# AlibabaResearch/efficientteacher

Hardware: AMD Instinct MI355X
Metric: SSOD images/sec (teacher+student step) YOLOv5l 640px (higher is better)
Workload: dtype bf16

## Files before the change

### efficientteacher_amd/_lib.py

```python
import ctypes
import os
from ctypes import c_char_p, c_double, c_float, c_int, c_int64, c_size_t, c_void_p

import torch

_HERE = os.path.dirname(os.path.abspath(__file__))
LIB_PATH = os.environ.get("ET_HIP_LIB") or os.path.join(_HERE, "libet_hip.so")

ET_F32, ET_BF16, ET_F16 = 0, 1, 2

P = c_void_p
SIGNATURES = {
    "et_build_arch": (c_char_p, []),
    "et_abi_version": (c_int, []),
    "et_nms_ssod_workspace_bytes": (c_int, [c_int, c_int, ctypes.POINTER(c_size_t)]),
    "et_nms_workspace_bytes": (c_int, [c_int, c_int, c_int, c_int, c_int, ctypes.POINTER(c_size_t)]),
    "et_nms": (c_int, [P, c_int, c_int, c_int, c_float, c_float, c_int, c_int, ctypes.c_uint64, ctypes.c_uint64, c_int,
                       c_float, c_int, P, P, P, P, P, c_size_t, P]),
    "et_nms_ssod": (c_int, [P, c_int, c_int, c_int, c_float, c_float, c_int, c_int, P, P, P, P, P, c_size_t, P]),
    "et_val_match": (c_int, [P, c_int, P, c_int, c_int, P, c_int, P, c_int, c_int, P, c_int, c_int, c_int, c_int64, c_int64,
                             P, P, P, P, P, P]),
    "et_val_ap_workspace_bytes": (c_int, [c_int, ctypes.POINTER(c_size_t)]),
    "et_val_ap": (c_int, [P, P, P, c_int64, P, c_int, c_int, P, P, P, P, P, c_size_t, P]),
    "et_detect_decode": (c_int, [P, c_int, c_int, c_int, c_int, c_int, c_int, c_int64, c_int64, c_int64, c_int64,
                                 P, c_float, P, c_int64, c_int64, P]),
    "et_ema_update": (c_int, [P, P, c_int64, c_float, c_float, P]),
    "et_adamw": (c_int, [P, P, P, P, P, c_int, c_int64, c_float, c_float, c_float, c_float, c_float, c_int, c_float, P, P]),
    "et_adamw_tick": (c_int, [P, c_float, c_float, P, P]),
    "et_adamw_dev": (c_int, [P, P, P, P, P, c_int, c_int64, c_float, c_float, c_float, c_float, c_float, P, c_float, P, P]),
    "et_sgd_nesterov": (c_int, [P, P, P, P, c_int, c_int64, c_float, c_float, c_float, c_int, c_float, P, P]),
    "et_cast_f32_to_lp": (c_int, [P, P, c_int, c_int64, P]),
    "et_scaler_check": (c_int, [P, c_int64, P, P]),
    "et_scaler_update": (c_int, [P, c_float, c_float, c_int, P]),
    "et_ema_update_dev": (c_int, [P, P, c_int64, P, P]),
    "et_sgd_nesterov_dev": (c_int, [P, P, P, P, c_int, c_int64, P, c_int, P, P]),
    "et_conv2d_stats_rows": (c_int, [c_int, c_int, c_int]),
    "et_conv2d_stats_rows_for": (c_int, [c_int] * 12),
    "et_conv2d_stats_adds_for": (c_int, [c_int] * 12),
    "et_conv2d_fwd": (c_int, [P, P, P, c_int] + [c_int] * 11 + [P, P, c_int, P, c_int, P, c_int, P, P]),
    "et_conv2d_dgrad": (c_int, [P, P, P, c_int] + [c_int] * 11 + [c_int, P, c_int, P, P]),
    "et_conv2d_dgrad_bn": (c_int, [P, P, P, c_int] + [c_int] * 10 + [P, c_int, P, c_int, P, P, c_int, P, c_int, P, P]),
    "et_conv2d_wgrad": (c_int, [P, P, P, c_int] + [c_int] * 11 + [P, P]),
    "et_conv2d_wgrad_grouped": (c_int, [P, c_int, c_int] + [c_int] * 9 + [P, P]),
    "et_weight_transpose_all": (c_int, [P, P, c_int, P, c_int, ctypes.c_longlong, P]),
    "et_weight_transpose": (c_int, [P, P, c_int, c_int, c_int, c_int, P]),
    "et_conv2d_kernel_name": (c_int, [c_int] * 13 + [c_char_p, c_int]),
    "et_env_knobs": (c_int, [c_char_p, c_int]),
    "et_colsum": (c_int, [P, c_int, c_int, c_int, c_int, P, P]),
    "et_bn_reduce_rows": (c_int, [c_int, c_int, c_int]),
    "et_bn_finalize": (c_int, [P, c_int, c_int, c_double, P, P, c_float, c_float, P, P, P, P, P, P, P, P]),
    "et_bn_eval_affine": (c_int, [c_int, P, P, P, P, c_float, P, P, P]),
    "et_bn_act_fwd": (c_int, [P, c_int, P, c_int, P, c_int, c_int, c_int, c_int, P, P, c_int, P]),
    "et_bn_act_fwd_sharded": (c_int, [P, c_int, P, c_int, P, c_int, c_int, c_int, c_int, P, c_int, c_double, P, P, c_float, c_float,
                                      P, P, P, P, P, P, c_int, P]),
    "et_bn_act_bwd_sharded": (c_int, [P, c_int, P, c_int, P, c_int, c_int, c_int, c_int, P, P, P, P, P, c_int, P, P, P, c_int, c_int, P]),
    "et_bn_act_bwd": (c_int, [P, c_int, P, c_int, P, c_int, c_int, c_int, c_int, P, P, P, P, P, c_int, P, P, P, P,
                              c_size_t, P]),
    "et_bn_act_bwd_from_partials": (c_int, [P, c_int, P, c_int, P, c_int, c_int, c_int, c_int, P, P, P, P, P, c_int, P, P, P,
                                            P, c_int, P, P]),
    "et_act_bwd": (c_int, [P, c_int, P, c_int, P, c_int, c_int, c_int, c_int, c_int, P]),
    "et_pack_input": (c_int, [P, P, c_int, c_int, c_int, c_int, c_int, P]),
    "et_pack_input_u8": (c_int, [P, P, c_int, c_int, c_int, c_int, c_int, c_float, P]),
    "et_maxpool5_fwd": (c_int, [P, c_int, P, c_int, P, c_int, c_int, c_int, c_int, c_int, P]),
    "et_maxpool5_bwd": (c_int, [P, c_int, P, P, c_int, P, c_int, c_int, c_int, c_int, c_int, c_int, P]),
    "et_upsample2x_fwd": (c_int, [P, c_int, P, c_int, c_int, c_int, c_int, c_int, c_int, P]),
    "et_upsample2x_bwd": (c_int, [P, c_int, P, c_int, c_int, c_int, c_int, c_int, c_int, c_int, P]),
    "et_strong_view_u8": (c_int, [P, P, c_int, c_int, c_int, P, P, P, P, c_int, P]),
    "et_mosaic4_u8": (c_int, [P, P, c_int, c_int, c_int, P]),
    "et_pseudo_label_transform": (c_int, [P, P, P, c_int, c_int, c_int, c_int, c_int, P, P, P]),
    "et_score_log_append": (c_int, [P, P, c_int, c_int, P, P, P, c_int64, P]),
    "et_yolo_loss": (c_int, [P, P]),
    "et_ota_workspace_bytes": (c_int, [c_int, c_int, c_int, c_int, ctypes.POINTER(c_size_t)]),
    "et_ota_assign": (c_int, [P, P, c_float, c_int, P, P, P]),
    "et_select_targets": (c_int, [P, P, c_int, P, P, c_int, c_int, P, P]),
    "et_scale_cast": (c_int, [P, P, c_int, c_int64, c_float, P, P]),
    "et_domain_focal": (c_int, [P, c_int, c_int, c_int64, c_int, c_float, P, c_int, P, P]),
    "et_scale_inplace": (c_int, [P, c_int, c_int64, c_float, P, P]),
    "et_v8_decode": (c_int, [P, c_int, P, c_int, c_int, c_int, c_int, c_int, c_int, c_int, c_float, c_float, P, c_int64, c_int64, P]),
    "et_tal_loss": (c_int, [P, P, P, P, P, P, P, c_int, c_int, c_int, c_int, c_int, c_float, c_float, c_float, P, P, P, P, P]),
    "et_tal_assign_workspace_bytes": (c_int, [c_int, c_int, c_int, ctypes.POINTER(c_size_t)]),
    "et_tal_assign": (c_int, [P, P, P, P, P, P, c_int, c_int, c_int, c_int, c_int, c_float, c_float, c_float, P, P, P, P, P, c_size_t, P]),
    "et_tal_targets_pad": (c_int, [P, c_int, c_int, c_int, c_float, c_float, P, P, P]),
    "et_tal_pseudo_split": (c_int, [P, P, P, P, c_int, c_int, c_int, c_int, c_int, c_int, c_float, c_float, P, P, P, P, P, P, P, P, P]),
    "et_tal_assigned_gt": (c_int, [P, c_int, c_int, c_int, P, P]),
    "et_tal_merge_pseudo": (c_int, [P, P, P, P, P, P, P, P, P, c_int, c_int, c_int, c_int, P, P, P, P]),
}



class WgradItem(ctypes.Structure):
    _fields_ = [("x", ctypes.c_void_p), ("dy", ctypes.c_void_p), ("dw", ctypes.c_void_p), ("ldx", ctypes.c_int),
                ("ldy", ctypes.c_int)]


class LossLevel(ctypes.Structure):
    _fields_ = [("p", P), ("dp", P), ("tobj_ws", P), ("sb", c_int64), ("sa", c_int64), ("sy", c_int64),
                ("sx", c_int64), ("ny", c_int), ("nx", c_int), ("anchors", c_float * 6), ("balance", c_float)]


class LossDesc(ctypes.Structure):
    _fields_ = [("dtype", c_int), ("B", c_int), ("na", c_int), ("nc", c_int), ("NT", c_int), ("nl", c_int),
                ("anchor_t", c_float), ("gr", c_float), ("cp", c_float), ("cn", c_float), ("cls_pw", c_float),
                ("obj_pw", c_float), ("box_w", c_float), ("obj_w", c_float), ("cls_w", c_float),
                ("pass_mask", c_int), ("ignore_obj", c_int), ("targets", P), ("acc_ws", P), ("out", P),
                ("ota_match", P), ("obj_channel", c_int), ("balance_dev", P), ("autobalance_ssi", c_int), ("fl_gamma", c_float), ("level", LossLevel * 4)]


_dll = None
_emulated = False
CALL_TIMER = None
_NO_LAUNCH = frozenset(n for n in (
    "et_build_arch", "et_abi_version", "et_nms_ssod_workspace_bytes", "et_nms_workspace_bytes", "et_conv2d_stats_rows", "et_conv2d_stats_rows_for",
    "et_conv2d_kernel_name", "et_env_knobs", "et_bn_reduce_rows", "et_ota_workspace_bytes", "et_tal_assign_workspace_bytes", "et_val_ap_workspace_bytes"))


class _TimedDll:

    def __init__(self, dll, timer):
        self._dll, self._timer, self._cache = dll, timer, {}

    def __getattr__(self, name):
        fn = self._cache.get(name)
        if fn is None:
            raw = getattr(self._dll, name)
            if name in _NO_LAUNCH or not name.startswith("et_"):
                fn = raw
            else:
                timer = self._timer

                def fn(*a, _raw=raw, _name=name):
                    tok = timer.begin(_name)
                    rc = _raw(*a)
                    timer.end(tok)
                    return rc
            self._cache[name] = fn
        return fn


class EtHipError(RuntimeError):
    pass


def _header_abi_version():
    import re
    with open(os.path.join(os.path.dirname(_HERE), "include", "et_hip.h")) as f:
        m = re.search(r"^#define\s+ET_ABI_VERSION\s+(\d+)", f.read(), re.M)
    if m is None:
        raise EtHipError("include/et_hip.h does not define ET_ABI_VERSION")
    return int(m.group(1))


ABI_VERSION = _header_abi_version()


def _declare(dll):
    for name, (res, args) in SIGNATURES.items():
        fn = getattr(dll, name)
        fn.restype = res
        fn.argtypes = args
    got = dll.et_abi_version()
    if got != ABI_VERSION:
        raise EtHipError(f"{getattr(dll, '_name', 'libet_hip.so')} has ABI version {got}, this binding needs {ABI_VERSION}: "
                         f"rebuild it (python -m efficientteacher_amd.csrc.build)")
    return dll


def load(path=None):
    global _dll
    if _dll is None:
        path = path or LIB_PATH
        if not os.path.exists(path):
            raise EtHipError(
                f"{path} not found: build the gfx950 kernels first "
                f"(python -m efficientteacher_amd.csrc.build).  There is no CPU fallback.")
        _dll = _declare(ctypes.CDLL(path))
    if CALL_TIMER is not None:
        w = getattr(CALL_TIMER, "_wrapped", None)
        if w is None or w._dll is not _dll:
            w = CALL_TIMER._wrapped = _TimedDll(_dll, CALL_TIMER)
        return w
    return _dll


def _use_library_for_tests(path, emulated):
    global _dll, _emulated
    _dll = _declare(ctypes.CDLL(path)) if path else None
    _emulated = bool(emulated) if path else False


def is_emulated():
    return _emulated


def check(rc, what):
    if rc != 0:
        raise EtHipError(f"{what} failed with code {rc}")


def ptr(t):
    if t is None:
        return None
    if not t.is_cuda and not _emulated:
        raise EtHipError("efficientteacher_amd kernels need CUDA/HIP tensors (got a CPU tensor); "
                         "there is no CPU fallback")
    return t.data_ptr()


_RAW_STREAM = getattr(torch._C, "_cuda_getCurrentRawStream", None)


def stream(t=None):
    if _emulated:
        return None
    if _RAW_STREAM is not None:
        idx = t.device.index if t is not None else None
        return _RAW_STREAM(torch.cuda.current_device() if idx is None else idx)
    return torch.cuda.current_stream(t.device if t is not None else None).cuda_stream
```

### efficientteacher_amd/autograd.py

```python
import torch
from torch.autograd import Function

from . import ops

ACT_CODE = {"silu": ops.ACT_SILU, "relu": ops.ACT_RELU, "none": ops.ACT_NONE}

FUSE_BN_BWD = True
FUSE_BN_BWD_K = 1
_RS_DGRAD = {}


def _dgrad_on_rs_tile(cs, x):
    key = (tuple(x.shape), x.dtype, cs.cinp, cs.coutp, cs.k, cs.stride, cs.pad)
    r = _RS_DGRAD.get(key)
    if r is None:
        N, H, W, _ = x.shape
        r = _RS_DGRAD[key] = cs.stride == 1 and ops.kernel_name("dgrad_full", x.dtype, N, H, W, cs.cinp, cs.coutp, cs.k, cs.stride,
                                                               cs.pad).startswith("conv_gemm_rs_kernel")
    return r


def _fuse_into(cs, bn, x=None):
    if bn is None:
        return None
    if FUSE_BN_BWD_K & (1 if cs.k == 1 else 2):
        return bn
    if cs.k > 1 and (FUSE_BN_BWD_K & 4) and x is not None and _dgrad_on_rs_tile(cs, x):
        return bn
    return None
SHARDED_BN = True


def _bn_train_fwd(x, w_lp, cs_stride, cs_pad, bs, act, residual=None, out=None):
    N, IH, IW, Cin = x.shape
    sh = None
    if SHARDED_BN and bs.sh_ld and ops.few_rows("fwd", x.dtype, N, IH, IW, Cin, w_lp.shape[0], w_lp.shape[1], cs_stride, cs_pad):
        sh = bs.acquire_fwd()
    if sh is not None:
        y = ops.conv2d_fwd(x, w_lp, cs_stride, cs_pad, shards=sh)
        N, OH, OW, _ = y.shape
        z, scale, shift, mean, invstd = ops.bn_act_fwd_sharded(y, sh, N * OH * OW, bs.gamma, bs.beta, bs.eps, bs.momentum, bs.rmean,
                                                               bs.rvar, act, residual=residual, out=out)
        return y, z, scale, shift, mean, invstd
    y, stats = ops.conv2d_fwd(x, w_lp, cs_stride, cs_pad, want_stats=True)
    N, OH, OW, _ = y.shape
    scale, shift, mean, invstd = ops.bn_finalize(stats, N * OH * OW, bs.gamma, bs.beta, bs.eps, bs.momentum, bs.rmean, bs.rvar)
    z = ops.bn_act_fwd(y, scale, shift, act, residual=residual, out=out)
    return y, z, scale, shift, mean, invstd


def _bn_sums(y, scale, shift, act, bs):
    return ops.BnBwdSums(y, scale, shift, act, slot=bs if (SHARDED_BN and bs.sh_ld) else None)


def _bn_train_bwd(dz, y, bs, scale, shift, mean, invstd, act, sums=None, out=None):
    part = sums.take(dz) if sums is not None else None
    if SHARDED_BN and bs.sh_ld and (isinstance(part, tuple) or (part is None and ops.few_reduce_rows(y))):
        sh = part if part is not None else bs.acquire_bwd()
        return ops.bn_act_bwd(dz, y, bs.gamma, scale, shift, mean, invstd, act, bs.ggamma, bs.gbeta, out=out, partial=part, shards=sh)
    return ops.bn_act_bwd(dz, y, bs.gamma, scale, shift, mean, invstd, act, bs.ggamma, bs.gbeta, out=out, partial=part)


GRAD_FORK = True

GRAD_READY_HOOK = None


class GradFork:

    def __init__(self):
        self.gb = None
        self.merged = False

    @staticmethod
    def split(x):
        if not (GRAD_FORK and torch.is_grad_enabled() and x.requires_grad):
            return x, x, None
        h = GradFork()
        a, b = _ForkFn.apply(x, h)
        return a, b, h

    @staticmethod
    def tap(b, fork):
        return b if fork is None else _TapFn.apply(b, fork)

    def take(self, shape, dtype):
        g = self.gb
        if g is None or tuple(g.shape) != tuple(shape) or g.dtype != dtype or g.dim() != 4 or g.stride(3) != 1:
            return None
        ld = g.stride(2)
        if not (ld >= g.shape[3] and g.stride(1) == ld * g.shape[2] and g.stride(0) == ld * g.shape[2] * g.shape[1]):
            return None
        return g


class _ForkFn(Function):
    @staticmethod
    def forward(ctx, x, holder):
        ctx.holder = holder
        return (x.as_strided(x.size(), x.stride(), x.storage_offset()), x.as_strided(x.size(), x.stride(), x.storage_offset()))

    @staticmethod
    def backward(ctx, ga, gb):
        h = ctx.holder
        merged = h.merged
        h.gb, h.merged = None, False
        if ga is None or gb is None:
            return (gb if ga is None else ga), None
        if merged:
            return ga, None
        return ga + gb, None


class _TapFn(Function):
    @staticmethod
    def forward(ctx, x, holder):
        ctx.holder = holder
        return x.as_strided(x.size(), x.stride(), x.storage_offset())

    @staticmethod
    def backward(ctx, g):
        ctx.holder.gb = g
        ctx.holder.merged = False
        return g, None


def _wgrad(x, dy, cs, *more_slots):
    hook = GRAD_READY_HOOK
    slots = (cs,) + more_slots

    def done():
        if hook is not None:
            for s in slots:
                hook(s)
    ops.WGRAD_QUEUE.submit(x, dy, cs.gw if not more_slots else _fused_gw(cs), cs.k, cs.stride, cs.pad,
                           on_done=done if hook is not None else None)


def _fused_gw(cs1):
    return cs1.gw.as_strided((2 * cs1.cout, 1, 1, cs1.cinp), (cs1.cinp, cs1.cinp, cs1.cinp, 1), cs1.gw.storage_offset())


class ConvBnActFn(Function):

    @staticmethod
    def forward(ctx, x, residual, wparam, cs, bs, act, nbt, dst=None, bn_in=None, bn_out=None, acc=None):
        ctx.w_needs_grad = wparam.requires_grad
        ctx.bn_in = bn_in if (bn_in is not None and cs.stride == 1 and residual is None) else None
        ctx.acc = acc
        if nbt is not None:
            nbt.add_(1)
        out = None if dst is None else dst[0][..., dst[1]:dst[1] + cs.coutp]
        y, z, scale, shift, mean, invstd = _bn_train_fwd(x, cs.w_lp, cs.stride, cs.pad, bs, act, residual=residual, out=out)
        ctx.cs, ctx.bs, ctx.act = cs, bs, act
        ctx.has_res = residual is not None
        ctx.x_needs_grad = x.requires_grad
        ctx.bn_mine = None
        if bn_out is not None and residual is None:
            ctx.bn_mine = _bn_sums(y, scale, shift, act, bs)
            bn_out.append(ctx.bn_mine)
        ctx.save_for_backward(x, y, scale, shift, mean, invstd)
        return z

    @staticmethod
    def backward(ctx, dz):
        x, y, scale, shift, mean, invstd = ctx.saved_tensors
        cs, bs = ctx.cs, ctx.bs
        dz = _dense_or_slice(dz)
        dy = _bn_train_bwd(dz, y, bs, scale, shift, mean, invstd, ctx.act, sums=ctx.bn_mine)
        if ctx.w_needs_grad:
            _wgrad(x, dy, cs)
        dx = None
        if ctx.x_needs_grad:
            wT = cs.transposed()
            into = ctx.acc.take(x.shape, dy.dtype) if (ctx.acc is not None and ctx.bn_in is None) else None
            if into is not None:
                dx = ops.conv2d_dgrad(dy, wT, (x.shape[1], x.shape[2]), cs.stride, cs.pad, out=into, accumulate=True)
                ctx.acc.merged = True
            else:
                dx = ops.conv2d_dgrad(dy, wT, (x.shape[1], x.shape[2]), cs.stride, cs.pad, bn=_fuse_into(cs, ctx.bn_in, x))
        return dx, (dz if ctx.has_res else None), None, None, None, None, None, None, None, None, None


class BottleneckFn(Function):

    @staticmethod
    def forward(ctx, x, w1, w2, cs1, bs1, cs2, bs2, act1, act2, nbt1, nbt2, dst=None, bn_in=None, bn_out=None):
        ctx.w_needs_grad = w1.requires_grad or w2.requires_grad
        ctx.bn_in = bn_in
        y1, h, *a1 = _bn_train_fwd(x, cs1.w_lp, cs1.stride, cs1.pad, bs1, act1)
        for nbt in (nbt1, nbt2):
            if nbt is not None:
                nbt.add_(1)
        out = None if dst is None else dst[0][..., dst[1]:dst[1] + cs2.coutp]
        y2, z, *a2 = _bn_train_fwd(h, cs2.w_lp, cs2.stride, cs2.pad, bs2, act2, residual=x, out=out)
        ctx.meta = (cs1, bs1, cs2, bs2, act1, act2)
        ctx.x_needs_grad = x.requires_grad
        ctx.bn_mine = None
        if bn_out is not None:
            ctx.bn_mine = _bn_sums(y2, a2[0], a2[1], act2, bs2)
            bn_out.append(ctx.bn_mine)
        ctx.save_for_backward(x, y1, h, y2, *a1, *a2)
        return z

    @staticmethod
    def backward(ctx, dz):
        x, y1, h, y2, s1, b1, m1, i1, s2, b2, m2, i2 = ctx.saved_tensors
        cs1, bs1, cs2, bs2, act1, act2 = ctx.meta
        dz = _dense_or_slice(dz)
        dy2 = _bn_train_bwd(dz, y2, bs2, s2, b2, m2, i2, act2, sums=ctx.bn_mine)
        if ctx.w_needs_grad:
            _wgrad(h, dy2, cs2)
        inner = _fuse_into(cs2, _bn_sums(y1, s1, b1, act1, bs1), h) if FUSE_BN_BWD else None
        dh = ops.conv2d_dgrad(dy2, cs2.transposed(), (h.shape[1], h.shape[2]), cs2.stride, cs2.pad, bn=inner)
        dy1 = _bn_train_bwd(dh, y1, bs1, s1, b1, m1, i1, act1, sums=inner)
        if ctx.w_needs_grad:
            _wgrad(x, dy1, cs1)
        dx = None
        if ctx.x_needs_grad:
            dx = ops.conv2d_dgrad(dy1, cs1.transposed(), (x.shape[1], x.shape[2]), cs1.stride, cs1.pad,
                                  residual=dz, bn=_fuse_into(cs1, ctx.bn_in, x))
        return (dx,) + (None,) * 13


def c3_stem_fusable(cs1, bs1, cs2, bs2):
    es = cs1.w_lp.element_size()
    return (cs1.k == 1 and cs2.k == 1 and cs1.stride == 1 and cs2.stride == 1 and cs1.cinp == cs2.cinp
            and cs1.coutp == cs1.cout and cs2.coutp == cs2.cout and cs1.cout == cs2.cout
            and cs2.w_lp.data_ptr() == cs1.w_lp.data_ptr() + cs1.w_lp.numel() * es
            and cs2.gw.data_ptr() == cs1.gw.data_ptr() + cs1.gw.numel() * 4
            and bs2.aff_off == bs1.aff_off + bs1.c and bs1.c == cs1.cout and bs2.c == cs2.cout
            and bs1.eps == bs2.eps and bs1.momentum == bs2.momentum)


def _fused_vec(a, b):
    return a.as_strided((a.numel() + b.numel(),), (1,), a.storage_offset())


class C3StemFn(Function):

    @staticmethod
    def forward(ctx, x, w1, w2, cs1, bs1, cs2, bs2, act, nbt1, nbt2, buf, bn_out=None):
        ctx.w_needs_grad = w1.requires_grad or w2.requires_grad
        c = cs1.cout
        wf = cs1.w_lp.as_strided((2 * c, 1, 1, cs1.cinp), (cs1.cinp, cs1.cinp, cs1.cinp, 1), cs1.w_lp.storage_offset())
        sh1 = sh2 = None
        if SHARDED_BN and bs1.sh_ld and bs2.sh_ld and ops.few_rows("fwd", x.dtype, x.shape[0], x.shape[1], x.shape[2], cs1.cinp, 2 * c, 1, 1, 0):
            sh1, sh2 = bs1.acquire_fwd(), bs2.acquire_fwd()
        for nbt in (nbt1, nbt2):
            if nbt is not None:
                nbt.add_(1)
        if sh1 is not None and sh2 is not None:
            y = ops.conv2d_fwd(x, wf, 1, 0, shards=sh1)
            N, H, W, _ = y.shape
            af = torch.empty((4, 2 * c), dtype=torch.float32, device=y.device)
            t = ops.bn_act_fwd_sharded(y[..., :c], sh1, N * H * W, bs1.gamma, bs1.beta, bs1.eps, bs1.momentum, bs1.rmean, bs1.rvar,
                                       act, out=buf[..., :c], aff=af[:, :c])[0]
            y2 = ops.bn_act_fwd_sharded(y[..., c:], sh2, N * H * W, bs2.gamma, bs2.beta, bs2.eps, bs2.momentum, bs2.rmean, bs2.rvar,
                                        act, out=buf[..., 2 * c:], aff=af[:, c:])[0]
            aff = (af[0], af[1], af[2], af[3])
        else:
            y, st = ops.conv2d_fwd(x, wf, 1, 0, want_stats=True)
            N, H, W, _ = y.shape
            aff = ops.bn_finalize(st, N * H * W, _fused_vec(bs1.gamma, bs2.gamma), _fused_vec(bs1.beta, bs2.beta), bs1.eps,
                                  bs1.momentum, _fused_vec(bs1.rmean, bs2.rmean), _fused_vec(bs1.rvar, bs2.rvar))
            t = ops.bn_act_fwd(y[..., :c], aff[0][:c], aff[1][:c], act, out=buf[..., :c])
            y2 = ops.bn_act_fwd(y[..., c:], aff[0][c:], aff[1][c:], act, out=buf[..., 2 * c:])
        ctx.meta = (cs1, bs1, cs2, bs2, act)
        ctx.x_needs_grad = x.requires_grad
        ctx.bn_mine = None
        if bn_out is not None:
            ctx.bn_mine = _bn_sums(y[..., :c], aff[0][:c], aff[1][:c], act, bs1)
            bn_out.append(ctx.bn_mine)
        ctx.save_for_backward(x, y, *aff)
        return t, y2

    @staticmethod
    def backward(ctx, dt, dy2):
        x, y, scale, shift, mean, invstd = ctx.saved_tensors
        cs1, bs1, cs2, bs2, act = ctx.meta
        c = cs1.cout
        N, H, W, _ = y.shape
        dy = torch.empty_like(y)
        halves = ((dt, slice(0, c), bs1), (dy2, slice(c, 2 * c), bs2))
        for g, sl, bs in halves:
            if g is None:
                dy[..., sl].zero_()
                continue
            g = _dense_or_slice(g)
            _bn_train_bwd(g, y[..., sl], bs, scale[sl], shift[sl], mean[sl], invstd[sl], act,
                          sums=ctx.bn_mine if sl.start == 0 else None, out=dy[..., sl])
        if ctx.w_needs_grad:
            _wgrad(x, dy, cs1, cs2)
        dx = None
        if ctx.x_needs_grad:
            wf = cs1.w_lp.as_strided((2 * c, 1, 1, cs1.cinp), (cs1.cinp, cs1.cinp, cs1.cinp, 1), cs1.w_lp.storage_offset())
            dx = ops.conv2d_dgrad(dy, ops.weight_transpose(wf), (x.shape[1], x.shape[2]), 1, 0)
        return (dx,) + (None,) * 11


class _GradDst:

    def __init__(self, p):
        self.shape, self.stride, self.dtype, self.device = tuple(p.shape), tuple(p.stride()), p.dtype, p.device
        self.span = ops._flat_span(p)
        self.buf = None
        self.written = [False, False]

    def flat(self, half, n):
        if self.buf is None:
            self.buf = torch.empty(self.span, dtype=self.dtype, device=self.device)
        cut = n * self.stride[0]
        self.written[half] = True
        return self.buf[:cut] if half == 0 else self.buf[cut:]


class BatchSplitFn(Function):
    @staticmethod
    def forward(ctx, p, n, holder):
        ctx.n, ctx.holder = n, holder
        return p[:n], p[n:]

    @staticmethod
    def backward(ctx, ga, gb):
        h, n = ctx.holder, ctx.n
        cut = n * h.stride[0]

        def is_slot(g, half):
            return (g is not None and h.buf is not None and h.written[half] and tuple(g.stride()) == h.stride
                    and g.data_ptr() == h.buf.data_ptr() + (cut * h.buf.element_size() if half else 0))
        if h.buf is None:
            h.buf = torch.empty(h.span, dtype=h.dtype, device=h.device)
        full = h.buf.as_strided(h.shape, h.stride)
        for half, g in ((0, ga), (1, gb)):
# ... 192 lines not shown
```

### efficientteacher_amd/csrc/conv.hip

```cpp
#include "et_device.h"
#include "../../include/et_hip.h"
#include <stdlib.h>
#include <stdio.h>
#include <string.h>
#include <type_traits>

typedef __attribute__((ext_vector_type(16))) float f32x16;
typedef __attribute__((ext_vector_type(8))) __bf16 bf16x8;
typedef __attribute__((ext_vector_type(8))) _Float16 f16x8;
typedef __attribute__((ext_vector_type(4))) unsigned int u32x4;
__device__ __forceinline__ u32x4 mk4(unsigned a, unsigned b, unsigned c, unsigned d) { u32x4 v = {a, b, c, d}; return v; }
__device__ __forceinline__ void et_pin_loaded(u32x4& v) {
#if defined(__HIP_DEVICE_COMPILE__)
    asm volatile("" : "+v"(v));
#endif
}

template <typename T, typename V> __device__ __forceinline__ f32x16 et_mfma32(const V a, const V b, const f32x16 c) {
    static_assert(sizeof(V) == 16, "8 x 16-bit operands");
    if constexpr (std::is_same<T, et_f16>::value)
        return __builtin_amdgcn_mfma_f32_32x32x16_f16(__builtin_bit_cast(f16x8, a), __builtin_bit_cast(f16x8, b), c, 0, 0, 0);
    else
        return __builtin_amdgcn_mfma_f32_32x32x16_bf16(__builtin_bit_cast(bf16x8, a), __builtin_bit_cast(bf16x8, b), c, 0, 0, 0);
}
// ... 1361 lines not shown
        const bool cok = c < g.Cout;
        cst[c] = (ep.scale && cok) ? ep.scale[c] : 1.0f;
        cst[BN + c] = (ep.bias && cok) ? ep.bias[c] : 0.0f;
        cst[2 * BN + c] = (FULL && ep.bn_y && cok) ? ep.bn_scale[c] : 1.0f;
        cst[3 * BN + c] = (FULL && ep.bn_y && cok) ? ep.bn_shift[c] : 0.0f;
    }

    int a_row[PER], a_lv[PER];
#pragma unroll
    for (int j = 0; j < PER; ++j) {
        a_row[j] = lrow + j * RPT;
        a_lv[j] = (lvec ^ lds_swz<BKV>(a_row[j])) * VEC;
    }
    et_rsrc rsX;
    if constexpr (BUF) {
        rsX = et_make_rsrc(X, (unsigned)(((size_t)(g.M - 1) * g.ldx + KC * 64) * sizeof(T)));
#pragma unroll
        for (int j = 0; j < PER; ++j) a_row[j] = (a_row[j] * g.ldx + a_lv[j]) * (int)sizeof(T);
    }
    const int ntiles = g.ntm;
    const int my_tiles = ((int)blockIdx.x < ntiles) ? (ntiles - 1 - (int)blockIdx.x) / (int)gridDim.x + 1 : 0;
    const int total = my_tiles * KC;
    int is_tile = blockIdx.x, is_kc = 0, is_slot = 0, issued = 0;
    auto issue = [&]() {
        if (stager) {
            u32x4* const wbase = ring + is_slot * CH_VEC + wave * 64;
            const int m0i = is_tile * BM;
            const unsigned soff = (unsigned)(((size_t)m0i * g.ldx + is_kc * 64) * sizeof(T));
#pragma unroll
            for (int j = 0; j < PER; ++j) {
                if constexpr (BUF) {
#if ET_S1_NT
                    et_bufdma16_nt(rsX, (unsigned)a_row[j], soff, wbase + j * DT);
#else
                    et_bufdma16(rsX, (unsigned)a_row[j], soff, wbase + j * DT);
#endif
                } else {
                    const int p = m0i + a_row[j];
                    const T* src = p < g.M ? X + ((size_t)p * g.ldx + is_kc * 64 + a_lv[j]) : ZERO;
#if ET_S1_NT
                    et_glds16_nt(src, wbase + j * DT);
#else
                    et_glds16(src, wbase + j * DT);
#endif
                }
            }
        }
        ++issued;
        if (++is_kc == KC) { is_kc = 0; is_tile += gridDim.x; }
        is_slot = is_slot + 1 == NS ? 0 : is_slot + 1;
    };
#pragma unroll
    for (int s = 0; s < NS - 1; ++s)
        if (issued < total) issue();

    u32x4 bw[TN][KC * 4];
#pragma unroll
    for (int tn = 0; tn < TN; ++tn) {
        const int co = wn * (32 * TN) + tn * 32 + l31;
        const bool cok = co < g.Cout;
        const T* wr = W + (size_t)(cok ? co : 0) * g.Cin + gk * VEC;
#pragma unroll
        for (int ks = 0; ks < KC * 4; ++ks) {
            bw[tn][ks] = *(const u32x4*)(wr + ks * 16);
            if (!cok) bw[tn][ks] = mk4(0, 0, 0, 0);
        }
    }
#pragma unroll
    for (int tn = 0; tn < TN; ++tn)
#pragma unroll
        for (int ks = 0; ks < KC * 4; ++ks) et_pin_loaded(bw[tn][ks]);
    __syncthreads();

    int abase[TM];
#pragma unroll
    for (int tm = 0; tm < TM; ++tm) {
        const int r = wm * (32 * TMW) + tm * 32 + l31;
        abase[tm] = (r * BKV + (gk ^ lds_swz<BKV>(r))) * 16;
    }

    EpiSums<TN> st;
    st.clear();
    st.cst = cst;
    st.cstride = BN;
    int rd = 0, q = 0;
    for (int i = 0; i < my_tiles; ++i) {
        const int m0 = ((int)blockIdx.x + i * (int)gridDim.x) * BM;
        f32x16 acc[TM][TN];
#pragma unroll
        for (int tm = 0; tm < TM; ++tm)
#pragma unroll
            for (int tn = 0; tn < TN; ++tn)
#pragma unroll
                for (int r = 0; r < 16; ++r) acc[tm][tn][r] = 0.f;
#pragma unroll
        for (int kc = 0; kc < KC; ++kc, ++q) {
            const int ahead = min(NS - 2, total - 1 - q);
            switch (ahead) {
#define ET_S1_WAIT(A) case A: et_wait_vmem_le_lds_read_done<((A) <= NS - 2 ? (A) : 0) * PER>(); break;
                ET_S1_WAIT(1) ET_S1_WAIT(2) ET_S1_WAIT(3) ET_S1_WAIT(4) ET_S1_WAIT(5) ET_S1_WAIT(6) ET_S1_WAIT(7)
                ET_S1_WAIT(8) ET_S1_WAIT(9) ET_S1_WAIT(10) ET_S1_WAIT(11) ET_S1_WAIT(12) ET_S1_WAIT(13) ET_S1_WAIT(14)
#undef ET_S1_WAIT
                default: et_wait_vmem_lds_read_done(); break;
            }
            __builtin_amdgcn_s_barrier();
            if (issued < total) issue();
            const char* const sa = (const char*)(ring + rd * CH_VEC);
            u32x4 af[2][TM];
#pragma unroll
            for (int tm = 0; tm < TM; ++tm) af[0][tm] = *(const u32x4*)(sa + abase[tm]);
#pragma unroll
            for (int kk = 0; kk < 4; ++kk) {
                const int cur = kk & 1;
                if (kk + 1 < 4) {
#pragma unroll
                    for (int tm = 0; tm < TM; ++tm) af[cur ^ 1][tm] = *(const u32x4*)(sa + (abase[tm] ^ ((kk + 1) * 32)));
                    __builtin_amdgcn_sched_barrier(0);
                }
#pragma unroll
                for (int tm = 0; tm < TM; ++tm)
#pragma unroll
                    for (int tn = 0; tn < TN; ++tn)
                        acc[tm][tn] = et_mfma32<T>(af[cur][tm], bw[tn][kc * 4 + kk], acc[tm][tn]);
            }
            rd = rd + 1 == NS ? 0 : rd + 1;
        }
        conv_epilogue<T, BM, BN, WM, WN, 16, MODE, true>(acc, slabs, Y, g, ep, 0, m0, 0, tid, lane, wm, wn, st);
    }
    if (ep.stats) {
        if (ep.stats_ld) conv_stats_add_sharded_wg<BN, WN, WM, MODE>(st, g, ep, tid, lane, wm, wn, (float*)ring);
        else conv_epilogue_write_stats<BN, WN, MODE>(st, g, ep, 0, lane, wn, (int)blockIdx.x * WM + wm, 0, (int)gridDim.x * WM);
    }
}
template <typename T, int KC, int WN, int TN, int WM, int TMW, int NS, int WGS, bool FULL>
__global__ __launch_bounds__(64 * WM * WN, WGS) void conv1x1_stream_kernel(const T* __restrict__ X, const T* __restrict__ W,
                                                                          T* __restrict__ Y, const T* __restrict__ ZERO,
                                                                          GatherGeom g, Epilogue ep) {
    conv1x1_stream_body<T, KC, WN, TN, WM, TMW, NS, WGS, FULL, true>(X, W, Y, ZERO, g, ep);
}
template <typename T, int KC, int WN, int TN, int WM, int TMW, int NS, int WGS, bool FULL>
__global__ __launch_bounds__(64 * WM * WN, WGS) void conv1x1_stream_flat_kernel(const T* __restrict__ X, const T* __restrict__ W,
                                                                               T* __restrict__ Y, const T* __restrict__ ZERO,
                                                                               GatherGeom g, Epilogue ep) {
    conv1x1_stream_body<T, KC, WN, TN, WM, TMW, NS, WGS, FULL, false>(X, W, Y, ZERO, g, ep);
}

#define STEM_TR 4
#define STEM_TC 64
#define STEM_PH 12
#define STEM_PITCH 132
#define STEM_PSLOTS (7 * 256)
#define STEM_WPITCH 37
#define STEM_WSLOTS (10 * 256)

struct StemArgs {
    const uint16_t* x; const uint16_t* w; uint16_t* y; const uint16_t* zero;
    int N, IH, IW, ldx, OH, OW, ldy, Cout;
    int trn, tcn, ntiles;
    const float* scale; const float* bias; int act;
    float* stats; int stat_rows;
    int stats_ld;
};

template <typename T, int ACT>
__global__ __launch_bounds__(256, 2) void conv_stem_kernel(StemArgs a) {
    __shared__ __attribute__((aligned(16))) u32x4 wl[STEM_WSLOTS];
    __shared__ __attribute__((aligned(16))) u32x4 pl[STEM_PSLOTS];
    const int tid = threadIdx.x, lane = tid & 63;
    const int wave = __builtin_amdgcn_readfirstlane(tid >> 6);
    const int l31 = lane & 31, hi = lane >> 5;

#pragma unroll
    for (int i = 0; i < STEM_WSLOTS / 256; ++i) {
        const int slot = i * 256 + tid;
        const int ch = slot / STEM_WPITCH, tap = slot - ch * STEM_WPITCH;
        const bool ok = ch < a.Cout && tap < 36;
        et_glds16(ok ? a.w + ((size_t)ch * 36 + tap) * 8 : a.zero, wl + i * 256 + wave * 64);
    }
    int s_dy[STEM_PSLOTS / 256], s_dx[STEM_PSLOTS / 256];
#pragma unroll
    for (int i = 0; i < STEM_PSLOTS / 256; ++i) {
        const int slot = i * 256 + tid;
        const int prow = slot / STEM_PITCH;
        s_dy[i] = prow < STEM_PH ? prow : -100000;
        s_dx[i] = slot - prow * STEM_PITCH;
    }
    float ssum[2][16], ssq[2][16];
#pragma unroll
    for (int cb = 0; cb < 2; ++cb)
#pragma unroll
        for (int r = 0; r < 16; ++r) { ssum[cb][r] = 0.f; ssq[cb][r] = 0.f; }
    float esc[2][2][8], ebi[2][2][8];
#pragma unroll
    for (int cb = 0; cb < 2; ++cb)
#pragma unroll
        for (int m = 0; m < 2; ++m)
#pragma unroll
            for (int e = 0; e < 8; ++e) {
                const int ch = cb * 32 + 8 * (2 * m + hi) + e;
                esc[cb][m][e] = (a.scale && ch < a.Cout) ? a.scale[ch] : 1.0f;
                ebi[cb][m][e] = (a.bias && ch < a.Cout) ? a.bias[ch] : 0.0f;
            }

    const u32x4* const wbase = wl + l31 * STEM_WPITCH + hi;
    const u32x4* const pbase = pl + (2 * wave) * STEM_PITCH + 2 * l31 + hi;

    auto stage_patch = [&](int tile) {
        const int tc = tile % a.tcn, t2 = tile / a.tcn;
        const int tr = t2 % a.trn, n = t2 / a.trn;
        const int iy0 = 2 * tr * STEM_TR - 2, ix0 = 2 * tc * STEM_TC - 2;
#pragma unroll
        for (int i = 0; i < STEM_PSLOTS / 256; ++i) {
            const int iy = iy0 + s_dy[i], ix = ix0 + s_dx[i];
            const bool ok = (unsigned)iy < (unsigned)a.IH && (unsigned)ix < (unsigned)a.IW;
            const uint16_t* src = ok ? a.x + (((size_t)n * a.IH + iy) * a.IW + ix) * a.ldx : a.zero;
            et_glds16(src, pl + i * 256 + wave * 64);
        }
    };
    if ((int)blockIdx.x < a.ntiles) stage_patch(blockIdx.x);
    for (int tile = blockIdx.x; tile < a.ntiles; tile += gridDim.x) {
        const int tc = tile % a.tcn, t2 = tile / a.tcn;
        const int tr = t2 % a.trn, n = t2 / a.trn;
        const int oy0 = tr * STEM_TR, ox0 = tc * STEM_TC;
        et_wait_vmem();
        __syncthreads();
        f32x16 acc[2][2];
#pragma unroll
        for (int cb = 0; cb < 2; ++cb)
#pragma unroll
            for (int pb = 0; pb < 2; ++pb)
#pragma unroll
                for (int r = 0; r < 16; ++r) acc[cb][pb][r] = 0.f;
#pragma unroll
        for (int ks = 0; ks < 18; ++ks) {
            u32x4 wf[2], pf[2];
#pragma unroll
            for (int cb = 0; cb < 2; ++cb) wf[cb] = wbase[cb * 32 * STEM_WPITCH + 2 * ks];
#pragma unroll
            for (int pb = 0; pb < 2; ++pb) pf[pb] = pbase[pb * 64 + (ks / 3) * STEM_PITCH + 2 * (ks % 3)];
#pragma unroll
            for (int cb = 0; cb < 2; ++cb)
#pragma unroll
                for (int pb = 0; pb < 2; ++pb)
                    acc[cb][pb] = et_mfma32<T>(wf[cb], pf[pb], acc[cb][pb]);
        }
        __syncthreads();
        if (tile + (int)gridDim.x < a.ntiles) stage_patch(tile + gridDim.x);
        const int oy = oy0 + wave;
#pragma unroll
        for (int pb = 0; pb < 2; ++pb) {
            const int ox = ox0 + pb * 32 + l31;
            const bool pok = oy < a.OH && ox < a.OW;
            uint16_t* const yp = a.y + (((size_t)n * a.OH + oy) * a.OW + ox) * a.ldy;
#pragma unroll
            for (int cb = 0; cb < 2; ++cb) {
                if (pok) {
#pragma unroll
                    for (int r = 0; r < 16; ++r) { const float raw = acc[cb][pb][r]; ssum[cb][r] += raw; ssq[cb][r] += raw * raw; }
                }
#pragma unroll
                for (int m = 0; m < 2; ++m) {
                    float lo4[4], hi4[4];
#pragma unroll
                    for (int e = 0; e < 4; ++e) {
                        const float q0 = acc[cb][pb][8 * m + e], q1 = acc[cb][pb][8 * m + 4 + e];
                        const float t = __shfl_xor(hi ? q0 : q1, 32);
                        lo4[e] = hi ? t : q0;
                        hi4[e] = hi ? q1 : t;
                    }
                    const int ch = cb * 32 + 8 * (2 * m + hi);
                    float v[8];
#pragma unroll
                    for (int e = 0; e < 8; ++e) {
                        float u = e < 4 ? lo4[e] : hi4[e - 4];
                        u = u * esc[cb][m][e] + ebi[cb][m][e];
                        if constexpr (ACT == ACT_SILU) u = u * __builtin_amdgcn_rcpf(1.0f + __expf(-u));
                        else if constexpr (ACT == ACT_RELU) u = fmaxf(u, 0.f);
                        v[e] = u;
                    }
                    if (pok && ch < a.Cout)
                        *(u32x4*)(yp + ch) = mk4(et_lp<T>::pack(v[0], v[1]), et_lp<T>::pack(v[2], v[3]), et_lp<T>::pack(v[4], v[5]), et_lp<T>::pack(v[6], v[7]));
                }
            }
        }
    }
    if (a.stats) {
        float* const red = (float*)wl;
        __syncthreads();
#pragma unroll
        for (int cb = 0; cb < 2; ++cb)
#pragma unroll
            for (int r = 0; r < 16; ++r) {
                float s1 = ssum[cb][r], s2 = ssq[cb][r];
#pragma unroll
                for (int m = 1; m < 32; m <<= 1) { s1 += __shfl_xor(s1, m); s2 += __shfl_xor(s2, m); }
                if (l31 == 0) {
                    const int ch = cb * 32 + 8 * (r >> 2) + 4 * hi + (r & 3);
                    red[(wave * 2 + 0) * 64 + ch] = s1;
                    red[(wave * 2 + 1) * 64 + ch] = s2;
                }
            }
        __syncthreads();
        if (tid < 128) {
            const int which = tid >> 6, ch = tid & 63;
            float t = 0.f;
#pragma unroll
            for (int w = 0; w < 4; ++w) t += red[(w * 2 + which) * 64 + ch];
            if (ch < a.Cout && a.stats_ld) {
                unsafeAtomicAdd(a.stats + ((size_t)(blockIdx.x % ET_BN_SHARDS) * 2 + which) * a.stats_ld + ch, t);
            } else if (ch < a.Cout) {
                for (int row = blockIdx.x; row < a.stat_rows; row += gridDim.x)
                    a.stats[((size_t)row * 2 + which) * a.Cout + ch] = row == (int)blockIdx.x ? t : 0.f;
            }
        }
    }
}

static int env_int(const char* name, int dflt) { const char* e = getenv(name); return e ? atoi(e) : dflt; }
static int device_cus() {
    static const int n_cu = [] { hipDeviceProp_t p; int d = 0; return (hipGetDevice(&d) == hipSuccess && hipGetDeviceProperties(&p, d) == hipSuccess && p.multiProcessorCount > 0) ? p.multiProcessorCount : 256; }();
    return n_cu;
}

static int try_launch_stem(const void* x, const void* w, void* y, int dtype, int N, int IH, int IW, int Cin, int ldx, int Cout,
                           int KH, int KW, int stride, int pad, int ldy, const float* scale, const float* bias, int act,
                           const void* residual, float* stats, int stats_ld, const void* zero16, hipStream_t s, bool launch) {
    if ((dtype != ET_BF16 && dtype != ET_F16) || KH != 6 || KW != 6 || stride != 2 || pad != 2 || Cin != 8 || Cout > 64 || Cout % 8 ||
        residual || !zero16)
        return 0;
    if (!launch) return 1;
    StemArgs a;
    a.x = (const uint16_t*)x; a.w = (const uint16_t*)w; a.y = (uint16_t*)y; a.zero = (const uint16_t*)zero16;
    a.N = N; a.IH = IH; a.IW = IW; a.ldx = ldx; a.Cout = Cout; a.ldy = ldy;
    a.OH = (IH + 2 * pad - KH) / stride + 1; a.OW = (IW + 2 * pad - KW) / stride + 1;
    a.trn = (a.OH + STEM_TR - 1) / STEM_TR; a.tcn = (a.OW + STEM_TC - 1) / STEM_TC;
    a.ntiles = N * a.trn * a.tcn;
    a.scale = scale; a.bias = bias; a.act = act; a.stats = stats; a.stats_ld = stats ? stats_ld : 0;
    a.stat_rows = (N * a.OH * a.OW + 63) / 64;
    int grid = env_int("ET_CONV_STEM_WGS", 2 * device_cus());
    if (grid < 1) grid = 1;
    if (grid > a.ntiles) grid = a.ntiles;
    if (stats && !stats_ld && grid > a.stat_rows) grid = a.stat_rows;
#define ET_STEM(T_) \
    do { \
        if (act == ACT_SILU) hipLaunchKernelGGL((conv_stem_kernel<T_, ACT_SILU>), dim3(grid), dim3(256), 0, s, a); \
        else if (act == ACT_RELU) hipLaunchKernelGGL((conv_stem_kernel<T_, ACT_RELU>), dim3(grid), dim3(256), 0, s, a); \
        else hipLaunchKernelGGL((conv_stem_kernel<T_, ACT_NONE>), dim3(grid), dim3(256), 0, s, a); \
    } while (0)
    if (dtype == ET_F16) ET_STEM(et_f16); else ET_STEM(uint16_t);
#undef ET_STEM
    return 1;
}

struct WgradGeom {
    int N, IH, IW, Cin, ldx;
    int QH, QW, P;
    int Cout, ldy;
    int isy, isx;
    int T, NC;
    int xcd;
    int Pper;
    int ntn, ntm, nsk;
    FastDiv dQW, dQH, dCin, dW1;
    int PP;
    int ident;
    int buf;
    signed char dy[CONV_MAX_TAPS], dx[CONV_MAX_TAPS];
};

template <typename T> struct Transposer;
template <> struct Transposer<uint16_t> {
    __device__ static __forceinline__ void run(const u32x4 (&in)[8], u32x4 (&out)[8]) {
        const uint32_t* s[8];
#pragma unroll
        for (int i = 0; i < 8; ++i) s[i] = (const uint32_t*)&in[i];
#pragma unroll
        for (int c = 0; c < 8; ++c) {
            uint32_t w[4];
#pragma unroll
            for (int j = 0; j < 4; ++j) {
                const uint32_t lo = s[2 * j][c >> 1], hi = s[2 * j + 1][c >> 1];
                w[j] = (c & 1) ? ((lo >> 16) | (hi & 0xffff0000u)) : ((lo & 0xffffu) | (hi << 16));
            }
            out[c] = mk4(w[0], w[1], w[2], w[3]);
        }
    }
};
template <> struct Transposer<et_f16> : Transposer<uint16_t> {};
template <> struct Transposer<float> {
    __device__ static __forceinline__ void run(const u32x4 (&in)[4], u32x4 (&out)[4]) {
        out[0] = mk4(in[0].x, in[1].x, in[2].x, in[3].x);
        out[1] = mk4(in[0].y, in[1].y, in[2].y, in[3].y);
        out[2] = mk4(in[0].z, in[1].z, in[2].z, in[3].z);
        out[3] = mk4(in[0].w, in[1].w, in[2].w, in[3].w);
    }
};

template <typename T, int BM, int BN>
__global__ __launch_bounds__(256) void conv_wgrad_kernel(const T* __restrict__ X, const T* __restrict__ DY,
                                                         float* __restrict__ DW, WgradGeom g) {
    constexpr int VEC = et_elem<T>::VEC, BKV = 8, WM = 2, WN = 2;
    constexpr int TM = BM / WM / 32, TN = BN / WN / 32;
    constexpr int GA = BM / VEC, GB = BN / VEC;
    constexpr int NBLK = (GA + GB) * BKV;
    constexpr int ITER = (NBLK + 255) / 256;
    constexpr int BKP = BKV * VEC;
    __shared__ __attribute__((aligned(16))) u32x4 lds[2][(BM + BN) * BKV];

    const int tid = threadIdx.x, lane = tid & 63, wave = tid >> 6;
    const int wm = wave / WN, wn = wave % WN;
    int bid = blockIdx.x;
    if (g.xcd) {
        const int nb = gridDim.x, q = nb >> 3, r = nb & 7, xcd = bid & 7, k = bid >> 3;
        bid = (xcd < r ? xcd * (q + 1) : r * (q + 1) + (xcd - r) * q) + k;
    }
    const int tx = bid % g.ntn, ty = (bid / g.ntn) % g.ntm, tz = bid / (g.ntn * g.ntm);
    const int n0 = tx * BN, m0 = ty * BM;
    const int pk_begin = tz * g.Pper;
    const int pk_end = min(g.P, pk_begin + g.Pper);

    bool isA[ITER], live[ITER], chan_ok[ITER];
    int grp[ITER], kvv[ITER], coff[ITER], tdy[ITER], tdx[ITER];
#pragma unroll
    for (int it = 0; it < ITER; ++it) {
        const int blk = tid + it * 256;
        live[it] = blk < NBLK;
        isA[it] = blk < GA * BKV;
        const int b2 = isA[it] ? blk : blk - GA * BKV;
        const int G = isA[it] ? GA : GB;
        grp[it] = b2 % G;
        kvv[it] = b2 / G;
        tdy[it] = tdx[it] = 0;
        if (isA[it]) {
            const int co = m0 + grp[it] * VEC;
            chan_ok[it] = co < g.Cout;
            coff[it] = co;
        } else {
            const int col = n0 + grp[it] * VEC;
            chan_ok[it] = col < g.NC;
            const uint32_t cc = chan_ok[it] ? col : 0;
            const uint32_t tap = fdiv(cc, g.dCin);
            coff[it] = cc - tap * g.Cin;
            tdy[it] = g.dy[tap];
            tdx[it] = g.dx[tap];
        }
    }

    f32x16 acc[TM][TN];
#pragma unroll
    for (int tm = 0; tm < TM; ++tm)
#pragma unroll
        for (int tn = 0; tn < TN; ++tn)
#pragma unroll
            for (int r = 0; r < 16; ++r) acc[tm][tn][r] = 0.f;

    u32x4 rawA[ITER][VEC], rawB[ITER][VEC];
    unsigned okA[ITER], okB[ITER];
    auto gload = [&](int pk0, u32x4 (&raw)[ITER][VEC], unsigned (&okm)[ITER]) {
#pragma unroll
        for (int it = 0; it < ITER; ++it) {
            okm[it] = 0u;
            if (!live[it]) continue;
            const int p0 = pk0 + kvv[it] * VEC;
            if (isA[it]) {
#pragma unroll
                for (int i = 0; i < VEC; ++i) {
                    const int p = p0 + i;
                    const bool ok = chan_ok[it] && p < pk_end;
                    raw[it][i] = *(const u32x4*)(DY + (ok ? (long long)p * g.ldy + coff[it] : 0));
// ... 124 lines not shown
#pragma unroll
    for (int j = 0; j < RA; ++j) {
        a_pl[j] = tid / SA + j * RPA;
        const int ls = (tid % SA) ^ tr_swz<SA>(a_pl[j]);
        a_co[j] = m0 + ls * 8;
        a_ok[j] = a_co[j] < g.Cout;
    }
    int b_pl[RB], b_ci[RB], b_dy[RB], b_dx[RB];
    bool b_ok[RB];
#pragma unroll
    for (int j = 0; j < RB; ++j) {
        b_pl[j] = tid / SB + j * RPB;
        const int ls = (tid % SB) ^ tr_swz<SB>(b_pl[j]);
        const int col = n0 + ls * 8;
        b_ok[j] = col < g.NC;
        const uint32_t cc = b_ok[j] ? col : 0;
        const uint32_t tap = fdiv(cc, g.dCin);
        b_ci[j] = cc - tap * g.Cin;
        b_dy[j] = g.dy[tap];
        b_dx[j] = g.dx[tap];
    }

    f32x16 acc[TM][TN];
#pragma unroll
    for (int tm = 0; tm < TM; ++tm)
#pragma unroll
        for (int tn = 0; tn < TN; ++tn)
#pragma unroll
            for (int r = 0; r < 16; ++r) acc[tm][tn][r] = 0.f;

    et_rsrc rsDY, rsX;
    unsigned a_vo[RA], b_vo[RB];
    if (g.buf) {
        rsDY = et_make_rsrc(DY, (unsigned)(((size_t)(pk_end - 1) * ldy + g.Cout) * 2));
        rsX = et_make_rsrc(X, (unsigned)(((size_t)(pk_end - 1) * ldx + g.NC) * 2));
#pragma unroll
        for (int j = 0; j < RA; ++j) a_vo[j] = a_ok[j] ? (unsigned)((a_pl[j] * ldy + a_co[j]) * 2) : 0x80000000u;
#pragma unroll
        for (int j = 0; j < RB; ++j) b_vo[j] = b_ok[j] ? (unsigned)((b_pl[j] * ldx + b_ci[j]) * 2) : 0x80000000u;
    }
    auto stage = [&](u32x4* dstA, u32x4* dstB, int pk0) {
        u32x4* const wa = dstA + wave * 64;
        u32x4* const wb = dstB + wave * 64;
        if (g.buf) {
            const unsigned sa = (unsigned)((size_t)pk0 * ldy * 2), sb = (unsigned)((size_t)pk0 * ldx * 2);
#pragma unroll
            for (int j = 0; j < RA; ++j) et_bufdma16(rsDY, a_vo[j], sa, wa + j * NT);
#pragma unroll
            for (int j = 0; j < RB; ++j) et_bufdma16(rsX, b_vo[j], sb, wb + j * NT);
            return;
        }
#pragma unroll
        for (int j = 0; j < RA; ++j) {
            const int p = pk0 + a_pl[j];
            const bool ok = a_ok[j] && p < pk_end;
            const uint16_t* src = ok ? DY + ((long long)p * ldy + a_co[j]) : ZERO;
            et_glds16(src, wa + j * NT);
        }
        if (g.ident) {
#pragma unroll
            for (int j = 0; j < RB; ++j) {
                const int p = pk0 + b_pl[j];
                const bool ok = b_ok[j] && p < pk_end;
                const uint16_t* src = ok ? X + ((long long)p * ldx + b_ci[j]) : ZERO;
                et_glds16(src, wb + j * NT);
            }
            return;
        }
#pragma unroll
        for (int j = 0; j < RB; ++j) {
            const int p = pk0 + b_pl[j];
            const uint32_t pp = min(p, g.P - 1);
            const uint32_t t1 = fdiv(pp, g.dQW), qx = pp - t1 * g.QW;
            const uint32_t n = fdiv(t1, g.dQH), qy = t1 - n * g.QH;
            const int iy = qy * g.isy + b_dy[j], ix = qx * g.isx + b_dx[j];
            const bool ok = b_ok[j] && p < pk_end && (unsigned)iy < (unsigned)g.IH && (unsigned)ix < (unsigned)g.IW;
            const uint16_t* src = ok ? X + ((((long long)n * g.IH + iy) * g.IW + ix) * ldx + b_ci[j]) : ZERO;
            et_glds16(src, wb + j * NT);
        }
    };

    const int fp = 8 * (lane >> 5) + ((lane & 15) >> 2);
    const int fc = 16 * ((lane >> 4) & 1) + 4 * (lane & 3);
    auto frag = [&](const char* tile, int slots, int ks, int c0, auto swz) -> s16x8 {
        s16x8 o;
#pragma unroll
        for (int r = 0; r < 2; ++r) {
            const int p = 16 * ks + 4 * r + fp;
            const int ch = c0 + fc;
            const int off = (p * slots + ((ch >> 3) ^ swz(p))) * 16 + (ch & 4) * 2;
            const s16x4 v = __builtin_amdgcn_ds_read_tr16_b64_v4i16((__attribute__((address_space(3))) s16x4*)(tile + off));
            o[4 * r + 0] = v[0]; o[4 * r + 1] = v[1]; o[4 * r + 2] = v[2]; o[4 * r + 3] = v[3];
        }
        return o;
    };
    auto mma = [&](const u32x4* bufA, const u32x4* bufB) {
        const char* ta = (const char*)bufA;
        const char* tb = (const char*)bufB;
#pragma unroll
        for (int ks = 0; ks < BKP / 16; ++ks) {
            s16x8 af[TM], bf[TN];
#pragma unroll
            for (int tm = 0; tm < TM; ++tm) af[tm] = frag(ta, SA, ks, wm * (BM / WM) + tm * 32, [](int p) { return tr_swz<SA>(p); });
#pragma unroll
            for (int tn = 0; tn < TN; ++tn) bf[tn] = frag(tb, SB, ks, wn * (BN / WN) + tn * 32, [](int p) { return tr_swz<SB>(p); });
#pragma unroll
            for (int tm = 0; tm < TM; ++tm)
#pragma unroll
                for (int tn = 0; tn < TN; ++tn)
                    acc[tm][tn] = et_mfma32<T>(af[tm], bf[tn], acc[tm][tn]);
        }
    };

    u32x4* const A0 = lds_raw;
    u32x4* const B0 = lds_raw + A_VEC;
    u32x4* const A1 = lds_raw + A_VEC + B_VEC;
    u32x4* const B1 = A1 + A_VEC;
    const int nchunks = (pk_end - pk_begin + BKP - 1) / BKP;
    if (nchunks > 0) stage(A0, B0, pk_begin);
    et_wait_vmem();
    __syncthreads();
    for (int c = 0; c < nchunks; ++c) {
        const bool odd = c & 1;
        if (c + 1 < nchunks) stage(odd ? A0 : A1, odd ? B0 : B1, pk_begin + (c + 1) * BKP);
        mma(odd ? A1 : A0, odd ? B1 : B0);
        et_wait_vmem();
        __syncthreads();
    }
    if (nchunks <= 0) return;
    const int l31 = lane & 31, hi = lane >> 5;
    if (m0 + BM <= g.Cout && n0 + BN <= g.NC) {
        float* const base = DW + ((size_t)(m0 + wm * (BM / WM) + 4 * hi) * g.NC + n0 + wn * (BN / WN) + l31);
#pragma unroll
        for (int tm = 0; tm < TM; ++tm)
#pragma unroll
            for (int r = 0; r < 16; ++r) {
                float* const rowp = base + (size_t)(tm * 32 + (r & 3) + 8 * (r >> 2)) * g.NC;
#pragma unroll
                for (int tn = 0; tn < TN; ++tn) atomicAdd(rowp + tn * 32, acc[tm][tn][r]);
            }
    } else {
#pragma unroll
        for (int tm = 0; tm < TM; ++tm)
#pragma unroll
            for (int r = 0; r < 16; ++r) {
                const int co = m0 + wm * (BM / WM) + tm * 32 + (r & 3) + 8 * (r >> 2) + 4 * hi;
#pragma unroll
                for (int tn = 0; tn < TN; ++tn) {
                    const int col = n0 + wn * (BN / WN) + tn * 32 + l31;
                    if (co < g.Cout && col < g.NC) atomicAdd(DW + ((size_t)co * g.NC + col), acc[tm][tn][r]);
                }
            }
    }
}

template <typename T, int BM, int BNC, int WM, int WN, int STRIDE = 1>
__global__ __launch_bounds__(64 * WM * WN) ET_WAVES_PER_EU(STRIDE == 1 ? 4 : 2) void conv_wgrad_rs_kernel(WgradGroup grp, const uint16_t* __restrict__ ZERO, WgradGeom g) {
    constexpr int NT = 64 * WM * WN, BKP = 64, BROWS = STRIDE == 1 ? 72 : 136;
    constexpr int TM = BM / WM / 32, TN = BNC / WN / 32;
    constexpr int SA = BM / 8, SB = BNC / 8;
    constexpr int RPA = NT / SA, RPB = NT / SB;
    constexpr int RA = BKP / RPA, RB = (BROWS + RPB - 1) / RPB;
    constexpr int A_VEC = BKP * SA, B_VEC = BROWS * SB;
    static_assert(RPA >= 1 && RPB >= 8 && TM >= 1 && TN >= 1 && (BROWS * SB) % 64 == 0 && RB * RPB > BKP, "staging passes");
    __shared__ __attribute__((aligned(16))) u32x4 lds_raw[2 * (A_VEC + B_VEC)];

    const int tid = threadIdx.x, lane = tid & 63, wave = tid >> 6;
    const int wm = wave / WN, wn = wave % WN;
    int bid = blockIdx.x;
    if (g.xcd) {
        const int nb = gridDim.x, q = nb >> 3, r = nb & 7, xcd = bid & 7, k = bid >> 3;
        bid = (xcd < r ? xcd * (q + 1) : r * (q + 1) + (xcd - r) * q) + k;
    }
    const int per_layer = g.ntn * g.ntm * g.nsk;
    const int layer = __builtin_amdgcn_readfirstlane(bid / per_layer);
    bid -= layer * per_layer;
    const uint16_t* __restrict__ X = grp.it[layer].x;
    const uint16_t* __restrict__ DY = grp.it[layer].dy;
    float* __restrict__ DW = grp.it[layer].dw;
    const int ldx = grp.it[layer].ldx, ldy = grp.it[layer].ldy;
    const int tx = bid % g.ntn, ty = (bid / g.ntn) % g.ntm, tz = bid / (g.ntn * g.ntm);
    const int nci = g.ntn / 3;
    const int jrow = tx / nci, c0 = (tx - jrow * nci) * BNC, m0 = ty * BM;
    const int dyr = jrow - 1;
    const int W1 = g.QW + 1;
    const int k_begin = tz * g.Pper;
    const int k_end = min(g.PP, k_begin + g.Pper);

    static_assert(BKP % RPA == 0 && BKP % RPB == 0 && RPA % 4 == 0 && RPB % (4 * STRIDE) == 0, "pieces are whole row groups; the swizzle repeats every 4 (8) rows");
    const int a_pl0 = tid / SA, b_pl0 = tid / SB;
    const int a_co = m0 + ((tid % SA) ^ tr_swz<SA>(a_pl0)) * 8;
    const int b_ci = c0 + ((tid % SB) ^ (STRIDE == 1 ? tr_swz<SB>(b_pl0) : tr_swz2<SB>(b_pl0))) * 8;
    const bool a_okc = a_co < g.Cout, b_okc = b_ci < g.Cin;

    constexpr int SPB = RPB / STRIDE;
    const int qa = RPA / W1, ra = RPA - qa * W1, qb = SPB / W1, rb = SPB - qb * W1;
    const int b_par = STRIDE == 1 ? 0 : (b_pl0 & 1);
    int a_yg, a_xp, b_yg, b_xp, b_qy;
    {
        const uint32_t sl = k_begin + a_pl0;
        a_yg = fdiv(sl, g.dW1);
        a_xp = sl - a_yg * W1;
        const uint32_t s1 = (STRIDE == 1 ? k_begin - 1 + b_pl0 : k_begin + (b_pl0 >> 1)) + W1;
        const uint32_t yg1 = fdiv(s1, g.dW1);
        b_xp = s1 - yg1 * W1;
        b_yg = (int)yg1 - 1;
        const int q1 = yg1 - fdiv(yg1, g.dQH) * g.QH;
        b_qy = q1 == 0 ? g.QH - 1 : q1 - 1;
    }

    f32x16 acc[3][TM][TN];
#pragma unroll
    for (int k = 0; k < 3; ++k)
#pragma unroll
        for (int tm = 0; tm < TM; ++tm)
#pragma unroll
            for (int tn = 0; tn < TN; ++tn)
#pragma unroll
                for (int r = 0; r < 16; ++r) acc[k][tm][tn][r] = 0.f;

    auto stage = [&](u32x4* dstA, u32x4* dstB, int k0) {
        u32x4* const wa = dstA + wave * 64;
        u32x4* const wb = dstB + wave * 64;
#pragma unroll
        for (int j = 0; j < RA; ++j) {
            const bool ok = a_okc && k0 + a_pl0 + j * RPA < k_end && a_xp < g.QW;
            const uint16_t* src = ok ? DY + ((size_t)(unsigned)((a_yg * g.QW + a_xp) * ldy + a_co)) : ZERO;
            et_glds16(src, wa + j * NT);
            a_xp += ra; a_yg += qa;
            if (a_xp >= W1) { a_xp -= W1; a_yg += 1; }
        }
        int yg = b_yg, xp = b_xp, qy = b_qy;
#pragma unroll
        for (int j = 0; j < RB; ++j) {
            if (j * RPB == BKP * STRIDE) { b_yg = yg; b_xp = xp; b_qy = qy; }
            if (RB * RPB > BROWS && j == RB - 1 && wave * 64 >= (BROWS - j * RPB) * SB) continue;
            bool ok;
            const uint16_t* src;
            if constexpr (STRIDE == 1) {
                ok = b_okc && yg >= 0 && k0 - 1 + b_pl0 + j * RPB < g.PP && b_pl0 + j * RPB < BROWS && xp < g.QW &&
                     (unsigned)(qy + dyr) < (unsigned)g.IH;
                src = ok ? X + ((size_t)(unsigned)((yg * g.QW + xp + dyr * g.IW) * ldx + b_ci)) : ZERO;
            } else {
                const int col = 2 * xp - 1 + b_par, iy = 2 * qy + dyr;
                ok = b_okc && yg >= 0 && k0 + ((b_pl0 + j * RPB) >> 1) < g.PP + 1 && b_pl0 + j * RPB < BROWS && xp <= g.QW &&
                     (unsigned)col < (unsigned)g.IW && (unsigned)iy < (unsigned)g.IH && yg < g.N * g.QH;
                src = ok ? X + ((size_t)(unsigned)(((2 * yg + dyr) * g.IW + col) * ldx + b_ci)) : ZERO;
            }
            et_glds16(src, wb + j * NT);
            int dq = qb;
            xp += rb;
            if (xp >= W1) { xp -= W1; dq += 1; }
            yg += dq; qy += dq;
            if (qy >= g.QH) qy -= g.QH;
        }
    };

    const int fp = 8 * (lane >> 5) + ((lane & 15) >> 2);
    const int fc = 16 * ((lane >> 4) & 1) + 4 * (lane & 3);
    int abase[TM], bbase[3][TN];
#pragma unroll
    for (int tm = 0; tm < TM; ++tm) {
        const int ch = wm * (BM / WM) + tm * 32 + fc;
        abase[tm] = (fp * SA + ((ch >> 3) ^ tr_swz<SA>(fp))) * 16 + (ch & 4) * 2;
    }
#pragma unroll
    for (int k = 0; k < 3; ++k)
#pragma unroll
        for (int tn = 0; tn < TN; ++tn) {
            const int ch = wn * (BNC / WN) + tn * 32 + fc;
            const int row = STRIDE * fp + k;
            bbase[k][tn] = (row * SB + ((ch >> 3) ^ (STRIDE == 1 ? tr_swz<SB>(row) : tr_swz2<SB>(row)))) * 16 + (ch & 4) * 2;
        }
    auto frag = [&](const char* tile, int base, int row_bytes, int ks) -> s16x8 {
        s16x8 o;
#pragma unroll
        for (int r = 0; r < 2; ++r) {
            const s16x4 v = __builtin_amdgcn_ds_read_tr16_b64_v4i16(
                (__attribute__((address_space(3))) s16x4*)(tile + base + (16 * ks + 4 * r) * row_bytes));
            o[4 * r + 0] = v[0]; o[4 * r + 1] = v[1]; o[4 * r + 2] = v[2]; o[4 * r + 3] = v[3];
        }
        return o;
    };
    auto mma = [&](const u32x4* bufA, const u32x4* bufB) {
        const char* ta = (const char*)bufA;
        const char* tb = (const char*)bufB;
#pragma unroll
        for (int ks = 0; ks < BKP / 16; ++ks) {
            s16x8 af[TM], bf[3][TN];
#pragma unroll
            for (int tm = 0; tm < TM; ++tm) af[tm] = frag(ta, abase[tm], SA * 16, ks);
#pragma unroll
            for (int k = 0; k < 3; ++k)
#pragma unroll
                for (int tn = 0; tn < TN; ++tn) bf[k][tn] = frag(tb, bbase[k][tn], STRIDE * SB * 16, ks);
#pragma unroll
            for (int k = 0; k < 3; ++k)
#pragma unroll
                for (int tm = 0; tm < TM; ++tm)
#pragma unroll
                    for (int tn = 0; tn < TN; ++tn)
                        acc[k][tm][tn] = et_mfma32<T>(af[tm], bf[k][tn], acc[k][tm][tn]);
        }
    };

    u32x4* const A0 = lds_raw;
// ... 618 lines not shown
                    if (eff(k) > eff(sk) + 0.1) sk = k;
            sk = max(1, min(sk, max_sk));
            int per = (g.PP + sk - 1) / sk;
            per = ((per + 63) / 64) * 64;
            sk = (g.PP + per - 1) / per;
            g.xcd = 1; g.Pper = per; g.nsk = sk;
            const dim3 grid(grp.n * g.ntn * g.ntm * sk);
            const uint16_t* z = (const uint16_t*)zero16;
            if (wp.rs_stride == 2) hipLaunchKernelGGL((conv_wgrad_rs_kernel<T, 128, 64, 2, 2, 2>), grid, dim3(256), 0, s, grp, z, g);
            else if (bm == 128) hipLaunchKernelGGL((conv_wgrad_rs_kernel<T, 128, 128, 2, 4>), grid, dim3(512), 0, s, grp, z, g);
            else hipLaunchKernelGGL((conv_wgrad_rs_kernel<T, 64, 64, 2, 2>), grid, dim3(256), 0, s, grp, z, g);
            return;
        }
    }
    const int tiles = grp.n * ((g.NC + bn - 1) / bn) * ((g.Cout + bm - 1) / bm);
    const int n_cu = device_cus();
    const int lds_kb = tr ? (bm + bn) / 4 : 64;
    int slots = tr ? max(1, min(160 / lds_kb, bm * bn <= 64 * 64 ? 5 : (bm * bn <= 128 * 64 ? 3 : 2))) : 2;
    const int cap = slots * n_cu;
    const int max_sk = max(1, g.P / (BKP * 25));
    auto eff = [&](int k) { const int b = tiles * k; return (double)b / ((double)((b + cap - 1) / cap) * cap); };
    int sk = max(1, min(cap / tiles, max_sk));
    if (eff(sk) < 0.8)
        for (int k = sk + 1; k <= min(max_sk, max(4, 2 * cap / tiles)); ++k)
            if (eff(k) > eff(sk) + 0.1) sk = k;
    sk = max(1, min(sk, max_sk));
    int per = (g.P + sk - 1) / sk;
    per = ((per + BKP - 1) / BKP) * BKP;
    sk = (g.P + per - 1) / per;
    g.xcd = 1;
    g.Pper = per;
    g.ntn = (g.NC + bn - 1) / bn; g.ntm = (g.Cout + bm - 1) / bm; g.nsk = sk;
    const dim3 block(256);
    if constexpr (sizeof(T) == 2) {
        if (tr) {
            const dim3 grid(grp.n * g.ntn * g.ntm * sk);
            const uint16_t* z = (const uint16_t*)zero16;
            g.buf = g.ident && env_int("ET_CONV_BUF_DMA", 1);
            for (int i = 0; i < grp.n && g.buf; ++i)
                if ((size_t)g.P * grp.it[i].ldx * 2 >= (1ull << 31) || (size_t)g.P * grp.it[i].ldy * 2 >= (1ull << 31)) g.buf = 0;
#define ET_WG(BM_, BN_, WM_, WN_) hipLaunchKernelGGL((conv_wgrad_tr_kernel<T, BM_, BN_, WM_, WN_>), grid, dim3(64 * WM_ * WN_), 0, s, grp, z, g)
            if (bm == 256) { if (bn == 256) ET_WG(256, 256, 2, 4); else if (bn == 128) ET_WG(256, 128, 4, 2); else ET_WG(256, 64, 4, 1); }
            else if (bm == 128) { if (bn == 256) ET_WG(128, 256, 2, 4); else if (bn == 128) ET_WG(128, 128, 2, 2); else ET_WG(128, 64, 2, 2); }
            else { if (bn == 256) ET_WG(64, 256, 1, 4); else if (bn == 128) ET_WG(64, 128, 2, 2); else ET_WG(64, 64, 2, 2); }
#undef ET_WG
            return;
        }
    }
    const dim3 grid(g.ntn * g.ntm * sk);
    for (int i = 0; i < grp.n; ++i) {
        const T* xx = (const T*)grp.it[i].x; const T* yy = (const T*)grp.it[i].dy;
        float* dw = grp.it[i].dw;
        g.ldx = grp.it[i].ldx; g.ldy = grp.it[i].ldy;
        if (tallM) {
            if (wideN) hipLaunchKernelGGL((conv_wgrad_kernel<T, 128, 128>), grid, block, 0, s, xx, yy, dw, g);
            else hipLaunchKernelGGL((conv_wgrad_kernel<T, 128, 64>), grid, block, 0, s, xx, yy, dw, g);
        } else {
            if (wideN) hipLaunchKernelGGL((conv_wgrad_kernel<T, 64, 128>), grid, block, 0, s, xx, yy, dw, g);
            else hipLaunchKernelGGL((conv_wgrad_kernel<T, 64, 64>), grid, block, 0, s, xx, yy, dw, g);
        }
    }
}

extern "C" int et_conv2d_wgrad_grouped(const et_wgrad_item* items, int n_items, int dtype, int N, int IH, int IW, int Cin,
                                       int Cout, int KH, int KW, int stride, int pad, const void* zero16,
                                       et_stream_t stream) {
    if (!items || n_items <= 0 || n_items > WGRAD_MAX_GROUP) return -1;
    if (KH * KW > CONV_MAX_TAPS || stride < 1 || N <= 0) return -2;
    const int vec = dtype == ET_F32 ? 4 : 8;
    if (Cin % vec || Cout % vec) return -2;
    WgradGroup grp;
    grp.n = n_items;
    for (int i = 0; i < n_items; ++i) {
        if (!items[i].x || !items[i].dy || !items[i].dw) return -1;
        grp.it[i].x = (const uint16_t*)items[i].x; grp.it[i].dy = (const uint16_t*)items[i].dy; grp.it[i].dw = items[i].dw;
        grp.it[i].ldx = items[i].ldx; grp.it[i].ldy = items[i].ldy;
    }
    for (int i = n_items; i < WGRAD_MAX_GROUP; ++i) grp.it[i] = grp.it[0];
    WgradGeom g;
    wgrad_geom(g, N, IH, IW, Cin, items[0].ldx, Cout, KH, KW, stride, pad, items[0].ldy);
    if (g.P <= 0) return 0;
    if (dtype == ET_F32) launch_wgrad<float>(grp, zero16, g, (hipStream_t)stream);
    else if (dtype == ET_BF16) launch_wgrad<uint16_t>(grp, zero16, g, (hipStream_t)stream);
    else if (dtype == ET_F16) launch_wgrad<et_f16>(grp, zero16, g, (hipStream_t)stream);
    else return -2;
    ET_CHECK_LAUNCH();
    return 0;
}

extern "C" int et_conv2d_wgrad(const void* x, const void* dy, float* dw, int dtype, int N, int IH, int IW, int Cin,
                               int ldx, int Cout, int KH, int KW, int stride, int pad, int ldy, const void* zero16,
                               et_stream_t stream) {
    const et_wgrad_item one{x, dy, dw, ldx, ldy};
    return et_conv2d_wgrad_grouped(&one, 1, dtype, N, IH, IW, Cin, Cout, KH, KW, stride, pad, zero16, stream);
}

extern "C" int et_weight_transpose(const void* w, void* wT, int dtype, int Cout, int taps, int Cin, et_stream_t stream) {
    if (!w || !wT) return -1;
    const long long n = (long long)Cout * taps * Cin;
    if (n <= 0) return -2;
    const dim3 grid(et_cdiv(n, 256)), block(256);
    if (dtype == ET_F32)
        hipLaunchKernelGGL((weight_transpose_kernel<float>), grid, block, 0, (hipStream_t)stream, (const float*)w, (float*)wT, Cout, taps, Cin, n);
    else if (dtype == ET_BF16 || dtype == ET_F16)
        hipLaunchKernelGGL((weight_transpose_kernel<uint16_t>), grid, block, 0, (hipStream_t)stream, (const uint16_t*)w, (uint16_t*)wT, Cout, taps, Cin, n);
    else return -2;
    ET_CHECK_LAUNCH();
    return 0;
}

extern "C" int et_weight_transpose_all(const void* w_arena, void* wT_arena, int dtype, const int* table, int n_layers,
                                       long long total_elems, et_stream_t stream) {
    if (!w_arena || !wT_arena || !table) return -1;
    if (n_layers <= 0 || total_elems <= 0) return -2;
    const dim3 grid(et_cdiv(total_elems, 256)), block(256);
    if (dtype == ET_F32)
        hipLaunchKernelGGL((weight_transpose_all_kernel<float>), grid, block, 0, (hipStream_t)stream, (const float*)w_arena,
                           (float*)wT_arena, table, n_layers, total_elems);
    else if (dtype == ET_BF16 || dtype == ET_F16) {
        if ((((uintptr_t)w_arena | (uintptr_t)wT_arena) & 15) == 0)
            hipLaunchKernelGGL(weight_transpose_all_tiled_kernel, dim3(96, n_layers), block, 0, (hipStream_t)stream,
                               (const uint16_t*)w_arena, (uint16_t*)wT_arena, table, n_layers);
        else
            hipLaunchKernelGGL((weight_transpose_all_kernel<uint16_t>), grid, block, 0, (hipStream_t)stream,
                               (const uint16_t*)w_arena, (uint16_t*)wT_arena, table, n_layers, total_elems);
    } else return -2;
    ET_CHECK_LAUNCH();
    return 0;
}

extern "C" int et_colsum(const void* x, int dtype, int P, int C, int ld, float* out, et_stream_t stream) {
    if (!x || !out) return -1;
    if (P <= 0 || C <= 0) return -2;
    const int rpb = 256;
    const dim3 grid((C + 255) / 256, (P + rpb - 1) / rpb), block(256);
    if (dtype == ET_F32) hipLaunchKernelGGL((colsum_kernel<float>), grid, block, 0, (hipStream_t)stream, (const float*)x, P, C, ld, rpb, out);
    else if (dtype == ET_BF16 || dtype == ET_F16) {
        const int CV = C / 8;
        const bool vec8 = C % 8 == 0 && ld % 8 == 0 && CV >= 1 && CV <= 256 && 256 % CV == 0 && (((uintptr_t)x) & 15) == 0;
        const int rpb2 = 256;
        if (dtype == ET_BF16) {
            if (vec8) hipLaunchKernelGGL((colsum_vec8_kernel<uint16_t>), dim3((P + rpb2 - 1) / rpb2), block, 0, (hipStream_t)stream, (const uint16_t*)x, P, CV, ld, rpb2, out);
            else hipLaunchKernelGGL((colsum_kernel<uint16_t>), grid, block, 0, (hipStream_t)stream, (const uint16_t*)x, P, C, ld, rpb, out);
        } else {
            if (vec8) hipLaunchKernelGGL((colsum_vec8_kernel<et_f16>), dim3((P + rpb2 - 1) / rpb2), block, 0, (hipStream_t)stream, (const et_f16*)x, P, CV, ld, rpb2, out);
            else hipLaunchKernelGGL((colsum_kernel<et_f16>), grid, block, 0, (hipStream_t)stream, (const et_f16*)x, P, C, ld, rpb, out);
        }
    }
    else return -2;
    ET_CHECK_LAUNCH();
    return 0;
}

extern "C" int et_conv2d_kernel_name(int op, int dtype, int N, int IH, int IW, int Cin, int Cout, int KH, int KW, int stride,
                                     int pad, int have_zero_page, int parity_class, char* buf, int buflen) {
    if (!buf || buflen < 8) return -1;
    if (KH * KW > CONV_MAX_TAPS || stride < 1 || N <= 0) return -2;
    const int eb = dtype == ET_F32 ? 4 : 2, vec = dtype == ET_F32 ? 4 : 8;
    if (op == 2) {
        WgradGeom g;
        wgrad_geom(g, N, IH, IW, Cin, Cin, Cout, KH, KW, stride, pad, Cout);
        wgrad_plan_name(plan_wgrad(g, eb, have_zero_page != 0), dtype, buf, buflen);
        return 0;
    }
    GatherGeom g;
    const bool full = op == 3 || op == 4;
    if (op == 3) op = 1;
    if (op == 4) op = 0;
    if (op == 0) {
        if (!full && try_launch_stem(nullptr, nullptr, nullptr, dtype, N, IH, IW, Cin, Cin, Cout, KH, KW, stride, pad, Cout, nullptr, nullptr, 0,
                                     nullptr, nullptr, 0, have_zero_page ? (const void*)buf : nullptr, nullptr, false)) {
            snprintf(buf, buflen, "conv_stem_kernel");
            return 0;
        }
        if (fwd_geom(g, N, IH, IW, Cin, Cin, Cout, KH, KW, stride, pad, Cout, vec)) return -2;
    } else if (op == 1) {
        if (stride > 2 || Cout % vec) return -2;
        const int py = parity_class / stride, px = parity_class % stride;
        if (py >= stride) return -2;
        if (dgrad_geom(g, py, px, N, IH, IW, Cin, Cin, Cout, KH, KW, stride, pad, Cout, vec)) return -2;
    } else return -2;
    plan_name(plan_gemm(g, eb, have_zero_page != 0, full), dtype, buf, buflen);
    return 0;
}

extern "C" int et_env_knobs(char* buf, int buflen) {
    static const char* names[] = {"ET_CONV_S1_WGS", "ET_CONV_STEM_WGS", "ET_CONV_BUF_DMA", "ET_BN_FIN_SMALL", "ET_STEP_GRAPH", "ET_WGRAD_STREAM",
                                  "ET_ALLREDUCE_CHUNK_MB", "ET_ALLREDUCE_DTYPE", "ET_RCCL_CHANNELS", "ET_DP_SINGLE_RANK", "ET_HIP_LIB"};
    if (!buf || buflen < 1) return -1;
    int off = 0;
    buf[0] = 0;
    for (const char* n : names) {
        const char* v = getenv(n);
        if (!v) continue;
        const int w = snprintf(buf + off, buflen - off, "%s=%s;", n, v);
        if (w < 0 || w >= buflen - off) return -3;
        off += w;
    }
    return 0;
}
```

### efficientteacher_amd/models/backbone/common.py

```python
import torch
import torch.nn as nn

from ... import ops
from ... import autograd as _ag
from ...autograd import BottleneckFn, C3StemFn, ConvBnActFn, JoinSlicesFn, SppfPoolFn, c3_stem_fusable


_ACTIVATIONS = {"silu": (nn.SiLU, None), "relu": (lambda: nn.ReLU(inplace=True), "relu")}


def get_activation(act=True):
    if isinstance(act, str):
        if act not in _ACTIVATIONS:
            raise AttributeError(f"activation '{act}' has no fused kernel (supported: {sorted(_ACTIVATIONS)})")
        make, name = _ACTIVATIONS[act]
        return make(), name
    if isinstance(act, nn.Module):
        return act, None
    return (nn.SiLU() if act is True else nn.Identity()), None


def autopad(k, p=None):
    if p is not None:
        return p
    return [x // 2 for x in k] if isinstance(k, (list, tuple)) else k // 2


def _act_code(m):
    if isinstance(m, nn.SiLU):
        return ops.ACT_SILU
    if isinstance(m, nn.ReLU):
        return ops.ACT_RELU
    if isinstance(m, nn.Identity):
        return ops.ACT_NONE
    raise NotImplementedError(f"activation {type(m).__name__} has no gfx950 kernel yet (SiLU / ReLU / Identity only)")


class Conv(nn.Module):
    def __init__(self, c1, c2, k=1, s=1, p=None, g=1, act=True):
        super().__init__()
        self.conv = nn.Conv2d(c1, c2, k, s, autopad(k, p), groups=g, bias=False)
        self.bn = nn.BatchNorm2d(c2)
        self.act, self.act_name = get_activation(act=act)

    def forward(self, x, residual=None, dst=None, bn_in=None, bn_out=None, acc=None):
        cs = getattr(self.conv, "_et_slot", None)
        if cs is None:
            raise RuntimeError("model state is not on the device arenas yet: move the Model to a GPU "
                               "(model.to('cuda')) before calling it -- there is no CPU path")
        bs = self.bn._et_slot
        act = _act_code(self.act)
        if self.bn.training:
            nbt = None if self._et_flat().bulk_nbt else self.bn.num_batches_tracked
            return ConvBnActFn.apply(x, residual, self.conv.weight, cs, bs, act, nbt, dst, bn_in, bn_out, acc)
        flat = self._et_flat()
        o = bs.aff_off
        out = None if dst is None else dst[0][..., dst[1]:dst[1] + cs.coutp]
        return ops.conv2d_fwd(x, cs.w_lp, cs.stride, cs.pad, scale=flat.eval_scale[o:o + bs.c],
                              bias=flat.eval_shift[o:o + bs.c], act=act, residual=residual, out=out)

    def forward_fuse(self, x):
        return self.forward(x)

    def _et_flat(self):
        return self.conv._et_flat_ref()


class Bottleneck(nn.Module):
    def __init__(self, c1, c2, shortcut=True, g=1, k=(1, 3), e=0.5, act=True):
        super().__init__()
        c_ = int(c2 * e)
        self.cv1 = Conv(c1, c_, k[0], 1, act=act)
        self.cv2 = Conv(c_, c2, k[1], 1, g=g, act=act)
        self.add = shortcut and c1 == c2

    def forward(self, x, dst=None, bn_in=None, bn_out=None):
        c1, c2 = self.cv1, self.cv2
        if (self.add and c1.bn.training and c2.bn.training and torch.is_grad_enabled() and c1.conv.stride[0] == 1
                and getattr(c1.conv, "_et_slot", None) is not None):
            bulk = c1._et_flat().bulk_nbt
            return BottleneckFn.apply(x, c1.conv.weight, c2.conv.weight, c1.conv._et_slot, c1.bn._et_slot,
                                      c2.conv._et_slot, c2.bn._et_slot, _act_code(c1.act), _act_code(c2.act),
                                      None if bulk else c1.bn.num_batches_tracked,
                                      None if bulk else c2.bn.num_batches_tracked, dst, bn_in, bn_out)
        if self.add or not (c1.bn.training and torch.is_grad_enabled() and _ag.FUSE_BN_BWD):
            return self.cv2(self.cv1(x), residual=x if self.add else None, dst=dst)
        mid = []
        h = self.cv1(x, bn_in=bn_in, bn_out=mid)
        return self.cv2(h, dst=dst, bn_in=mid[0] if mid else None, bn_out=bn_out)


class C3(nn.Module):
    def __init__(self, c1, c2, n=1, shortcut=True, g=1, e=0.5, act=True):
        super().__init__()
        c_ = int(c2 * e)
        if act == 'relu_silu':
            act, last_act = 'relu', 'silu'
        elif act == 'silu':
            act, last_act = 'silu', 'silu'
        elif act == 'relu_lrelu':
            act, last_act = 'relu', 'lrelu'
        elif act == 'relu_hswish':
            act, last_act = 'relu', 'hard_swish'
        else:
            last_act = act
        self.cv1 = Conv(c1, c_, 1, 1, act=act)
        self.cv2 = Conv(c1, c_, 1, 1, act=act)
        self.cv3 = Conv(2 * c_, c2, 1, act=last_act)
        self.m = nn.Sequential(*[Bottleneck(c_, c_, shortcut, g, e=1.0, act=act) for _ in range(n)])

    def forward(self, x, dst=None):
        N, H, W, _ = x.shape
        c_ = self.cv2.conv.out_channels
        c1s, c2s = getattr(self.cv1.conv, "_et_slot", None), getattr(self.cv2.conv, "_et_slot", None)
        last = len(self.m) - 1
        if (c1s is not None and self.cv1.bn.training and self.cv2.bn.training and torch.is_grad_enabled()
                and len(self.m) > 0 and c3_stem_fusable(c1s, self.cv1.bn._et_slot, c2s, self.cv2.bn._et_slot)):
            buf = torch.empty((N, H, W, 3 * c_), dtype=x.dtype, device=x.device)
            bulk = self.cv1._et_flat().bulk_nbt
            fuse = _ag.FUSE_BN_BWD
            hand = [] if fuse else None
            t, y2 = C3StemFn.apply(x, self.cv1.conv.weight, self.cv2.conv.weight, c1s, self.cv1.bn._et_slot, c2s,
                                   self.cv2.bn._et_slot, _act_code(self.cv1.act),
                                   None if bulk else self.cv1.bn.num_batches_tracked,
                                   None if bulk else self.cv2.bn.num_batches_tracked, buf, hand)
            for i, b in enumerate(self.m):
                nxt = [] if (fuse and i != last) else None
                t = b(t, dst=(buf, c_) if i == last else None, bn_in=hand[0] if hand else None, bn_out=nxt)
                hand = nxt
            return self.cv3(JoinSlicesFn.apply((buf[..., c_:],), t, y2), dst=dst)
        if (c1s is not None and not self.cv1.bn.training and not self.cv2.bn.training and not torch.is_grad_enabled() and len(self.m) > 0
                and c3_stem_fusable(c1s, self.cv1.bn._et_slot, c2s, self.cv2.bn._et_slot)
                and _act_code(self.cv1.act) == _act_code(self.cv2.act)):
            flat = self.cv1._et_flat()
            o = self.cv1.bn._et_slot.aff_off
            buf = torch.empty((N, H, W, 2 * c_), dtype=x.dtype, device=x.device)
            wf = c1s.w_lp.as_strided((2 * c_, 1, 1, c1s.cinp), (c1s.cinp, c1s.cinp, c1s.cinp, 1), c1s.w_lp.storage_offset())
            ops.conv2d_fwd(x, wf, 1, 0, scale=flat.eval_scale[o:o + 2 * c_], bias=flat.eval_shift[o:o + 2 * c_],
                           act=_act_code(self.cv1.act), out=buf)
            t = buf[..., :c_]
            for i, b in enumerate(self.m):
                t = b(t, dst=(buf, 0) if i == last else None)
            return self.cv3(buf, dst=dst)
        buf = torch.empty((N, H, W, 2 * c_), dtype=x.dtype, device=x.device)
        y2 = self.cv2(x, dst=(buf, c_))
        train = self.cv1.bn.training and torch.is_grad_enabled() and _ag.FUSE_BN_BWD and len(self.m) > 0
        hand = [] if train else None
        t = self.cv1(x, bn_out=hand)
        for i, b in enumerate(self.m):
            nxt = [] if (train and i != last) else None
            t = b(t, dst=(buf, 0) if i == last else None, bn_in=hand[0] if hand else None, bn_out=nxt)
            hand = nxt
        if torch.is_grad_enabled() and (t.requires_grad or y2.requires_grad):
            cat = JoinSlicesFn.apply((buf,), t, y2)
        else:
            cat = buf
        return self.cv3(cat, dst=dst)


class C2f(nn.Module):
    def __init__(self, c1, c2, n=1, shortcut=False, g=1, e=0.5, act=True):
        super().__init__()
        self.c = int(c2 * e)
        if self.c % 8:
            raise NotImplementedError("C2f hidden width must be a multiple of 8 channels (16-byte NHWC vectors)")
        self.cv1 = Conv(c1, 2 * self.c, 1, 1, act=act)
        self.cv2 = Conv((2 + n) * self.c, c2, 1, act=act)
        self.m = nn.ModuleList(Bottleneck(self.c, self.c, shortcut, g, k=(3, 3), e=1.0, act=act) for _ in range(n))

    def forward(self, x):
        N, H, W, _ = x.shape
        c, n = self.c, len(self.m)
        buf = torch.empty((N, H, W, (2 + n) * c), dtype=x.dtype, device=x.device)
        y = self.cv1(x, dst=(buf, 0))
        parts = [y]
        t = y[..., c:]
        for i, m in enumerate(self.m):
            t = m(t, dst=(buf, (2 + i) * c))
            parts.append(t)
        if torch.is_grad_enabled() and any(p.requires_grad for p in parts):
            return self.cv2(JoinSlicesFn.apply((buf,), *parts))
        return self.cv2(buf)


class SPPF(nn.Module):
    def __init__(self, c1, c2, k=5, act=True):
        super().__init__()
        if k != 5:
            raise NotImplementedError("the SPPF pooling kernel is specialised for k=5 (every shipped config)")
        c_ = c1 // 2
        if act == 'relu_silu':
            act, last_act = 'relu', 'silu'
        elif act == 'relu_lrelu':
            act, last_act = 'relu', 'lrelu'
        elif act == 'relu_hswish':
            act, last_act = 'relu', 'hard_swish'
        else:
            last_act = act
        self.cv1 = Conv(c1, c_, 1, 1, act=act)
        self.cv2 = Conv(c_ * 4, c2, 1, 1, act=last_act)
        self.m = nn.MaxPool2d(kernel_size=k, stride=1, padding=k // 2)

    def forward(self, x):
        cs = getattr(self.cv1.conv, "_et_slot", None)
        if cs is None or cs.coutp != self.cv1.conv.out_channels:
            return self.cv2(SppfPoolFn.apply(self.cv1(x)))
        N, H, W, _ = x.shape
# ... 12 lines not shown
```

### efficientteacher_amd/models/backbone/yolov5_backbone.py

```python
import torch.nn as nn

from ...autograd import GradFork

from ...utils.general import make_divisible
from .common import C3, SPPF, Conv


STAGE_EVENTS = None


def _mark_stage(name, t):
    if STAGE_EVENTS is not None and t.is_cuda and t.requires_grad:
        import torch
        e = torch.cuda.Event()
        e.record()
        STAGE_EVENTS[name] = e


class YoloV5BackBone(nn.Module):
    supports_concat_dst = True

    def __init__(self, cfg):
        super(YoloV5BackBone, self).__init__()
        self.gd = cfg.Model.depth_multiple
        self.gw = cfg.Model.width_multiple
        self.channels_out = {'stage1': 64, 'stage2_1': 128, 'stage2_2': 128, 'stage3_1': 256, 'stage3_2': 256,
                             'stage4_1': 512, 'stage4_2': 512, 'stage5': 1024, 'spp': 1024, 'csp1': 1024,
                             'conv1': 1024}
        self.re_channels_out()
        if cfg.Model.Backbone.activation == 'SiLU':
            CONV_ACT, C_ACT = 'silu', 'silu'
        elif cfg.Model.Backbone.activation == 'ReLU':
            CONV_ACT, C_ACT = 'relu', 'relu'
        else:
            CONV_ACT, C_ACT = 'hard_swish', 'relu_hswish'
        c = self.channels_out
        self.stage1 = Conv(3, c['stage1'], 6, 2, 2, 1, CONV_ACT)
        self.stage2_1 = Conv(c['stage1'], c['stage2_1'], 3, 2, None, 1, CONV_ACT)
        self.stage2_2 = C3(c['stage2_1'], c['stage2_2'], self.get_depth(3), True, 1, 0.5, C_ACT)
        self.stage3_1 = Conv(c['stage2_2'], c['stage3_1'], 3, 2, None, 1, CONV_ACT)
        self.stage3_2 = C3(c['stage3_1'], c['stage3_2'], self.get_depth(6), True, 1, 0.5, C_ACT)
        self.stage4_1 = Conv(c['stage3_2'], c['stage4_1'], 3, 2, None, 1, CONV_ACT)
        self.stage4_2 = C3(c['stage4_1'], c['stage4_2'], self.get_depth(9), True, 1, 0.5, C_ACT)
        self.stage5_1 = Conv(c['stage4_2'], c['stage5'], 3, 2, None, 1, CONV_ACT)
        self.stage5_2 = C3(c['stage5'], c['csp1'], self.get_depth(3), True, 1, 0.5, C_ACT)
        self.sppf = SPPF(c['csp1'], c['spp'], 5, CONV_ACT)
        self.out_shape = {'C3_size': c['stage3_2'], 'C4_size': c['stage4_2'], 'C5_size': c['conv1']}

    def forward(self, x, dst_c3=None, dst_c4=None):
        x1 = self.stage1(x)
        _mark_stage("p1", x1)
        x21 = self.stage2_1(x1)
        x22 = self.stage2_2(x21)
        _mark_stage("p2", x22)
        x31 = self.stage3_1(x22)
        c3, c3n, f3 = GradFork.split(self.stage3_2(x31, dst=dst_c3))
        _mark_stage("p3", c3)
        x41 = self.stage4_1(c3, acc=f3)
        c4, c4n, f4 = GradFork.split(self.stage4_2(x41, dst=dst_c4))
        _mark_stage("p4", c4)
        x51 = self.stage5_1(c4, acc=f4)
        x5 = self.stage5_2(x51)
        return GradFork.tap(c3n, f3), GradFork.tap(c4n, f4), self.sppf(x5)

    def get_depth(self, n):
        return max(round(n * self.gd), 1) if n > 1 else n

    def get_width(self, n):
        return make_divisible(n * self.gw, 8)

    def re_channels_out(self):
        for k, v in self.channels_out.items():
            self.channels_out[k] = self.get_width(v)
```

### efficientteacher_amd/models/detector/yolo.py

```python
import copy
import logging

import torch
import torch.nn as nn

from ... import _lib, ops
from ...flat_state import FlatState
from ...utils.torch_utils import initialize_weights
from ..backbone import build_backbone
from ..head import build_head
from ..head.yolov5_head import Detect
from ..neck import build_neck

LOGGER = logging.getLogger(__name__)


def check_anchor_order(m):
    a = m.anchors.prod(-1).view(-1)
    da = a[-1] - a[0]
    ds = m.stride[-1] - m.stride[0]
    if da.sign() != ds.sign():
        m.anchors[:] = m.anchors.flip(0)


class Model(nn.Module):
    def __init__(self, cfg='yolov5s.yaml'):
        super().__init__()
        self.cfg = cfg
        self.backbone = build_backbone(cfg)
        self.neck = build_neck(cfg)
        self.head = build_head(cfg)
        self.names = cfg.Dataset.names
        self.inplace = self.cfg.Model.inplace
        self.model_type = 'yolov5'
        self.export = False
        self._build_extra(cfg)
        self.check_head()
        initialize_weights(self)
        self._flat = None
        self._compute_dtype = torch.float32
        self._deterministic = bool(getattr(cfg.Model, "deterministic_bn", False)) if hasattr(cfg, "Model") else False

    def _build_extra(self, cfg):
        pass

    def check_head(self):
        m = self.head
        from ..head.yolov8_head import YoloV8Detect
        if isinstance(m, YoloV8Detect):
            m.inplace = self.inplace
            self.stride = torch.Tensor(m.stride)
            m.initialize_biases()
            self.model_type = 'yolox'
            return
        if not isinstance(m, Detect):
            raise NotImplementedError
        m.inplace = self.inplace
        m.stride = torch.tensor([8., 16., 32.])
        m.anchors /= m.stride.view(-1, 1, 1)
        check_anchor_order(m)
        self.stride = m.stride
        m.initialize_biases()

    def info(self, verbose=False, img_size=640):
        n_p = sum(x.numel() for x in self.parameters())
        n_g = sum(x.numel() for x in self.parameters() if x.requires_grad)
        LOGGER.info(f"Model summary: {len(list(self.modules()))} layers, {n_p} parameters, {n_g} gradients")

    def fuse(self):
        return self

    def half(self):
        return self.set_compute_dtype(torch.bfloat16)

    def float(self):
        return self.set_compute_dtype(torch.float32)

    def flat_state(self):
        if self._flat is None:
            raise RuntimeError("model is not on a GPU: call model.to('cuda') first (no CPU path)")
        return self._flat

    def set_compute_dtype(self, dtype):
        if dtype not in (torch.float32, torch.bfloat16, torch.float16):
            raise TypeError(dtype)
        self._compute_dtype = dtype
        self.rebuild_flat()
        return self

    def set_deterministic(self, flag=True):
        self._deterministic = bool(flag)
        self.rebuild_flat()
        return self

    def rebuild_flat(self):
        for m in self.modules():
            m.__dict__.pop("_et_slot", None)
            m.__dict__.pop("_et_flat_ref", None)
        self._flat = None
        ps = list(self.parameters())
        on_dev = all(p.is_cuda for p in ps) or (_lib.is_emulated() and all(p.device.type == 'cpu' for p in ps))
        if ps and on_dev and all(p.dtype == torch.float32 for p in ps):
            req = [p.requires_grad for p in ps]
            self._flat = FlatState(self, self._compute_dtype, deterministic=getattr(self, "_deterministic", False))
            for p, r in zip(ps, req):
                p.requires_grad_(r)
                if not r:
                    p.grad = None
        return self

    def _apply(self, fn, *a, **k):
        super()._apply(fn, *a, **k)
        self.rebuild_flat()
        return self

    def __deepcopy__(self, memo):
        flat, slots = self._flat, []
        for m in self.modules():
            slots.append((m, m.__dict__.pop("_et_slot", None), m.__dict__.pop("_et_flat_ref", None)))
        self._flat = None
        try:
            new = self.__class__.__new__(self.__class__)
            memo[id(self)] = new
            new.__dict__ = copy.deepcopy(self.__dict__, memo)
        finally:
            self._flat = flat
            for m, s, r in slots:
                if s is not None:
                    m._et_slot = s
                if r is not None:
                    m._et_flat_ref = r
        new.rebuild_flat()
        return new

    def __reduce_ex__(self, protocol):
        from ...utils.checkpoint import reduce_model
        return reduce_model(self, protocol)

    def load_state_dict(self, *a, **k):
        r = super().load_state_dict(*a, **k)
        if self._flat is not None:
            self._flat.mark_weights_changed()
        return r

    def zero_grad(self, set_to_none=False):
        if self._flat is not None:
            self._flat.zero_grad()
        else:
            super().zero_grad(set_to_none)

    def forward(self, x, augment=False, profile=False, visualize=False):
        return self._forward_once(x, profile, visualize)

    def _features(self, x):
        flat = self.flat_state()
        flat.prepare_forward(self.training)
        if not all(t.dim() == 4 and t.shape[1] <= 8 for t in (x if isinstance(x, (list, tuple)) else (x,))):
            raise ValueError("expected an NCHW image batch (B, 3, H, W), or a list of such batches of one shape")
        x8 = ops.pack_input(x, self._compute_dtype, norm_scale=getattr(self, "input_norm_scale", 255.0))
        slots = None
        if (hasattr(self.neck, "concat_slots") and getattr(self.backbone, "supports_concat_dst", False)
                and x8.shape[1] % 32 == 0 and x8.shape[2] % 32 == 0):
            slots = self.neck.concat_slots(x8.shape[0], x8.shape[1] // 8, x8.shape[2] // 8, x8.dtype, x8.device)
        if slots is None:
            return self.neck(self.backbone(x8))
        (b3, o3), (b4, o4) = slots
        c3, c4, c5 = self.backbone(x8, dst_c3=(b3, o3), dst_c4=(b4, o4))
        return self.neck((c3, c4, c5), cat_bufs=(b3, b4))

    def _forward_once(self, x, profile=False, visualize=False):
        return self.head(self._features(x))
```

### efficientteacher_amd/ops.py

```python
import torch

from . import _lib
from ._lib import ET_BF16, ET_F16, ET_F32

ACT_NONE, ACT_SILU, ACT_RELU = 0, 1, 2


class KernelTimer:

    def __init__(self):
        self.rows = []
        self.shapes = []

    def span(self, tag, flops, launches=1, nbytes=0, shape=None):
        a, b = torch.cuda.Event(enable_timing=True), torch.cuda.Event(enable_timing=True)
        self.rows.append((tag, flops, launches, nbytes, a, b))
        self.shapes.append(shape)
        return a, b

    def summary(self):
        agg = {}
        for tag, fl, n, nb, a, b in self.rows:
            ms = a.elapsed_time(b)
            t = agg.setdefault(tag, dict(ms=0.0, flops=0.0, launches=0, bytes=0.0))
            t["ms"] += ms; t["flops"] += fl; t["launches"] += n; t["bytes"] += nb
        return agg


TIMER = None
SCOPE = None


class FamilyTimer:

    FAMILY = {
        "et_conv2d_fwd": "gather_gemm", "et_conv2d_dgrad": "gather_gemm", "et_conv2d_dgrad_bn": "gather_gemm",
        "et_conv2d_wgrad": "wgrad", "et_conv2d_wgrad_grouped": "wgrad",
        "et_bn_finalize": "bn", "et_bn_act_fwd": "bn", "et_bn_act_fwd_sharded": "bn", "et_bn_act_bwd_sharded": "bn", "et_bn_act_bwd": "bn", "et_bn_act_bwd_from_partials": "bn", "et_act_bwd": "bn",
        "et_nms": "nms_loss_pl", "et_nms_ssod": "nms_loss_pl", "et_detect_decode": "nms_loss_pl", "et_pseudo_label_transform": "nms_loss_pl",
        "et_select_targets": "nms_loss_pl", "et_yolo_loss": "nms_loss_pl", "et_ota_assign": "nms_loss_pl", "et_score_log_append": "nms_loss_pl",
        "et_scale_cast": "nms_loss_pl", "et_domain_focal": "nms_loss_pl", "et_scale_inplace": "nms_loss_pl", "et_v8_decode": "nms_loss_pl",
        "et_tal_loss": "nms_loss_pl", "et_tal_assign": "nms_loss_pl", "et_colsum": "nms_loss_pl", "et_tal_pseudo_split": "nms_loss_pl", "et_tal_targets_pad": "nms_loss_pl",
        "et_tal_assigned_gt": "nms_loss_pl", "et_tal_merge_pseudo": "nms_loss_pl",
        "et_sgd_nesterov": "optimizer_ema", "et_sgd_nesterov_dev": "optimizer_ema", "et_adamw": "optimizer_ema", "et_ema_update": "optimizer_ema",
        "et_ema_update_dev": "optimizer_ema", "et_cast_f32_to_lp": "optimizer_ema", "et_scaler_check": "optimizer_ema", "et_scaler_update": "optimizer_ema", "et_weight_transpose": "optimizer_ema",
        "et_weight_transpose_all": "optimizer_ema", "et_bn_eval_affine": "optimizer_ema",
    }

    def __init__(self):
        self.rows = []

    def begin(self, name):
        fam = self.FAMILY.get(name, "pool_upsample_pack")
        if fam == "gather_gemm":
            fam = "gather_gemm_teacher" if SCOPE == "teacher" else "gather_gemm_student"
        a, b = torch.cuda.Event(enable_timing=True), torch.cuda.Event(enable_timing=True)
        a.record()
        return (fam, torch.cuda.current_stream().cuda_stream, a, b)

    def end(self, tok):
        tok[3].record()
        self.rows.append(tok)

    def summary(self):
        out = {}
        for fam, sid, a, b in self.rows:
            d = out.setdefault(sid, {})
            d[fam] = d.get(fam, 0.0) + a.elapsed_time(b)
        return out


def kernel_name(op, dtype, N, IH, IW, Cin, Cout, k, stride, pad, parity_class=0, zero_page=True):
    import ctypes
    buf = ctypes.create_string_buffer(256)
    code = {"fwd": 0, "dgrad": 1, "wgrad": 2, "dgrad_full": 3, "fwd_res": 4}[op]
    dt = _ET_OF[dtype]
    _lib.check(_lib.load().et_conv2d_kernel_name(code, dt, N, IH, IW, Cin, Cout, k, k, stride, pad, int(bool(zero_page)),
                                                 parity_class, buf, 256), "et_conv2d_kernel_name")
    return buf.value.decode()


def stats_rows(op, dtype, N, IH, IW, Cin, Cout, k, stride, pad, zero_page=True):
    dt = _ET_OF[dtype]
    rows = _lib.load().et_conv2d_stats_rows_for({"fwd": 0, "dgrad_bn": 1, "fwd_res": 2}[op], dt, N, IH, IW, Cin, Cout, k, k, stride, pad, int(bool(zero_page)))
    if rows <= 0:
        raise _lib.EtHipError(f"et_conv2d_stats_rows_for failed with code {rows}")
    return rows


def stats_adds(op, dtype, N, IH, IW, Cin, Cout, k, stride, pad, zero_page=True):
    dt = _ET_OF[dtype]
    n = _lib.load().et_conv2d_stats_adds_for({"fwd": 0, "dgrad_bn": 1, "fwd_res": 2}[op], dt, N, IH, IW, Cin, Cout, k, k, stride, pad, int(bool(zero_page)))
    if n <= 0:
        raise _lib.EtHipError(f"et_conv2d_stats_adds_for failed with code {n}")
    return n


SHARD_MAX_ADDS = 12800
_FEW_ROWS = {}


def few_rows(op, dtype, N, IH, IW, Cin, Cout, k, stride, pad):
    key = (op, dtype, N, IH, IW, Cin, Cout, k, stride, pad)
    r = _FEW_ROWS.get(key)
    if r is None:
        r = _FEW_ROWS[key] = stats_adds(op, dtype, N, IH, IW, Cin, Cout, k, stride, pad)
    return r <= SHARD_MAX_ADDS


def few_reduce_rows(y):
    N, H, W, C = y.shape
    return _lib.load().et_bn_reduce_rows(N * H * W, C, et_dtype(y)) <= SHARD_MAX_ADDS


def env_knobs():
    import ctypes
    buf = ctypes.create_string_buffer(1024)
    _lib.check(_lib.load().et_env_knobs(buf, 1024), "et_env_knobs")
    return buf.value.decode()


_ZERO_PAGES = {}


def zero_page(device):
    z = _ZERO_PAGES.get(device)
    if z is None:
        z = _ZERO_PAGES[device] = torch.zeros(256, dtype=torch.uint8, device=device)
    return z


_BN_TOTALS = {}


def bn_totals_scratch(device):
    key = (device, torch.cuda.current_stream(device).cuda_stream if device.type == "cuda" else 0)
    z = _BN_TOTALS.get(key)
    if z is None:
        z = _BN_TOTALS[key] = torch.zeros(2 * 2048 + 32, dtype=torch.float64, device=device)
    return z


_ET_OF = {torch.float32: ET_F32, torch.bfloat16: ET_BF16, torch.float16: ET_F16}
LP_DTYPES = (torch.bfloat16, torch.float16)


def et_dtype(t):
    try:
        return _ET_OF[t.dtype]
    except KeyError:
        raise TypeError(f"unsupported dtype {t.dtype} (float32 = parity mode, bfloat16 = performance mode, float16 = the "
                        "reference's AMP recipe)") from None


def _nhwc(x):
    assert x.dim() == 4 and x.stride(3) == 1, "NHWC tensor with contiguous channels expected"
    ld = x.stride(2)
    assert x.stride(1) == ld * x.shape[2] and x.stride(0) == ld * x.shape[2] * x.shape[1], \
        "pixels must be dense over the pixel stride"
    return ld


def conv_out_hw(ih, iw, k, s, p):
    return (ih + 2 * p - k) // s + 1, (iw + 2 * p - k) // s + 1


def conv2d_fwd(x, w, stride, pad, *, scale=None, bias=None, act=ACT_NONE, residual=None, out=None, want_stats=False, shards=None):
    N, IH, IW, Cin = x.shape
    Cout, KH, KW, Cin2 = w.shape
    assert Cin == Cin2 and w.is_contiguous() and w.dtype == x.dtype
    OH, OW = conv_out_hw(IH, IW, KH, stride, pad)
    lib = _lib.load()
    if out is None:
        out = torch.empty((N, OH, OW, Cout), dtype=x.dtype, device=x.device)
    assert out.shape == (N, OH, OW, Cout)
    stats, stats_ld = None, 0
    if shards is not None:
        assert not want_stats
        stats, stats_ld = shards
    if want_stats:
        rows = stats_rows("fwd_res" if residual is not None else "fwd", x.dtype, N, IH, IW, Cin, Cout, KH, stride, pad)
        stats = torch.empty((rows, 2, Cout), dtype=torch.float32, device=x.device)
    ldr = _nhwc(residual) if residual is not None else 0
    ev = TIMER.span(kernel_name("fwd_res" if residual is not None else "fwd", x.dtype, N, IH, IW, Cin, Cout, KH, stride, pad), 2.0 * N * OH * OW * Cout * Cin * KH * KW,
                    nbytes=(x.numel() + N * OH * OW * Cout + w.numel()) * x.element_size(),
                    shape=("fwd", N, IH, IW, Cin, Cout, KH, stride)) if TIMER else None
    if ev:
        ev[0].record()
    _lib.check(lib.et_conv2d_fwd(_lib.ptr(x), _lib.ptr(w), _lib.ptr(out), et_dtype(x), N, IH, IW, Cin, _nhwc(x),
                                 Cout, KH, KW, stride, pad, _nhwc(out), _lib.ptr(scale), _lib.ptr(bias), act,
                                 _lib.ptr(residual), ldr, _lib.ptr(stats), stats_ld, _lib.ptr(zero_page(x.device)),
                                 _lib.stream(x)), "et_conv2d_fwd")
    if ev:
        ev[1].record()
    return (out, stats) if want_stats else out


class WgradQueue:

    def __init__(self):
        import os
        self.group = 8
        self.stale = 20
        self.pending = {}
        self.last = {}
        self.tick = 0
        self._cb_armed = False
        self.use_side = int(os.environ.get("ET_WGRAD_STREAM", "1") or 0)
        self._side = {}
        self._dirty = set()

    def side_stream(self, dev):
        s = self._side.get(dev)
        if s is None:
            s = self._side[dev] = torch.cuda.Stream(device=dev)
        return s

    def reset(self):
        self.pending.clear()
        self.last.clear()
        self._cb_armed = False
        self.join()

    def submit(self, x, dy, dw, ksize, stride, pad, on_done=None):
        if self.group <= 1 or x.dtype not in LP_DTYPES:
            conv2d_wgrad(x, dy, dw, ksize, stride, pad)
            if on_done is not None:
                on_done()
            return
        if not self._cb_armed:
            try:
                torch.autograd.Variable._execution_engine.queue_callback(self.flush)
                self._cb_armed = True
            except RuntimeError:
                conv2d_wgrad(x, dy, dw, ksize, stride, pad)
                if on_done is not None:
                    on_done()
                return
        key = (tuple(x.shape), tuple(dy.shape), ksize, stride, pad, x.device)
        self.tick += 1
        for k in [k for k, t in self.last.items() if k != key and self.tick - t > self.stale]:
            self._flush_key(k)
        lst = self.pending.setdefault(key, [])
        lst.append((x, dy, dw, on_done))
        self.last[key] = self.tick
        if len(lst) >= self.group:
            self._flush_key(key)

    def _flush_key(self, key):
        lst = self.pending.pop(key, None)
        self.last.pop(key, None)
        if not lst:
            return
        xs, dys, ksize, stride, pad, dev = key
        items = [(a, b, c) for a, b, c, _ in lst]
        if dev.type == "cuda" and (self.use_side == 1 or (self.use_side == 2 and ksize == 1) or (self.use_side == 3 and ksize > 1)):
            main, side = torch.cuda.current_stream(dev), self.side_stream(dev)
            side.wait_stream(main)
            with torch.cuda.stream(side):
                conv2d_wgrad_grouped(items, ksize, stride, pad)
                for a, b, _ in items:
                    a.record_stream(side)
                    b.record_stream(side)
                for _, _, _, cb in lst:
                    if cb is not None:
                        cb()
            self._dirty.add(dev)
            return
        conv2d_wgrad_grouped(items, ksize, stride, pad)
        for _, _, _, cb in lst:
            if cb is not None:
                cb()

    def join(self):
        for dev in self._dirty:
            torch.cuda.current_stream(dev).wait_stream(self._side[dev])
        self._dirty.clear()

    def flush(self):
        self._cb_armed = False
        for key in list(self.pending.keys()):
            self._flush_key(key)
        self.join()


WGRAD_QUEUE = WgradQueue()


def conv2d_wgrad_grouped(items, ksize, stride, pad):
    x0, dy0, dw0 = items[0]
    N, IH, IW, Cin = x0.shape
    _, OH, OW, Cout = dy0.shape
    arr = (_lib.WgradItem * len(items))()
    for i, (x, dy, dw) in enumerate(items):
        assert x.shape == x0.shape and dy.shape == dy0.shape and x.dtype == dy.dtype == x0.dtype
        assert dw.dtype == torch.float32 and dw.is_contiguous() and dw.shape == (Cout, ksize, ksize, Cin)
        arr[i].x, arr[i].dy, arr[i].dw = _lib.ptr(x), _lib.ptr(dy), _lib.ptr(dw)
        arr[i].ldx, arr[i].ldy = _nhwc(x), _nhwc(dy)
    ev = TIMER.span(kernel_name("wgrad", x0.dtype, N, IH, IW, Cin, Cout, ksize, stride, pad),
                    2.0 * len(items) * N * OH * OW * Cout * Cin * ksize * ksize, 1,
                    nbytes=len(items) * ((N * IH * IW * Cin + N * OH * OW * Cout) * x0.element_size() + 8 * Cout * Cin * ksize * ksize),
                    shape=("wgrad", N, IH, IW, Cin, Cout, ksize, stride)) if TIMER else None
    if ev:
        ev[0].record()
    _lib.check(_lib.load().et_conv2d_wgrad_grouped(arr, len(items), et_dtype(x0), N, IH, IW, Cin, Cout, ksize, ksize,
                                                   stride, pad, _lib.ptr(zero_page(x0.device)), _lib.stream(x0)),
               "et_conv2d_wgrad_grouped")
    if ev:
        ev[1].record()


def weight_transpose(w):
    Cout, KH, KW, Cin = w.shape
    wt = torch.empty((Cin, KH, KW, Cout), dtype=w.dtype, device=w.device)
    _lib.check(_lib.load().et_weight_transpose(_lib.ptr(w), _lib.ptr(wt), et_dtype(w), Cout, KH * KW, Cin,
                                               _lib.stream(w)), "et_weight_transpose")
    return wt


def weight_transpose_all(w_arena, wT_arena, table, total):
    _lib.check(_lib.load().et_weight_transpose_all(_lib.ptr(w_arena), _lib.ptr(wT_arena), et_dtype(w_arena),
                                                   _lib.ptr(table), table.shape[0], int(total), _lib.stream(w_arena)),
               "et_weight_transpose_all")


class BnBwdSums:
    __slots__ = ("y", "scale", "shift", "act", "partial", "dz_ptr", "slot")

    def __init__(self, y, scale, shift, act, slot=None):
        self.y, self.scale, self.shift, self.act, self.slot = y, scale, shift, act, slot
        self.partial, self.dz_ptr = None, None

    def take(self, dz):
        p = self.partial if (self.partial is not None and dz.data_ptr() == self.dz_ptr) else None
        self.partial, self.dz_ptr = None, None
        return p


def conv2d_dgrad(dy, wT, in_hw, stride, pad, *, out=None, accumulate=False, residual=None, bn=None):
    N, OH, OW, Cout = dy.shape
    Cin, KH, KW, Cout2 = wT.shape
    assert Cout == Cout2 and wT.dtype == dy.dtype
    IH, IW = in_hw
    assert conv_out_hw(IH, IW, KH, stride, pad) == (OH, OW)
    if out is None:
        assert not accumulate
        out = torch.empty((N, IH, IW, Cin), dtype=dy.dtype, device=dy.device)
    if bn is not None and stride == 1 and not accumulate and bn.y.shape == out.shape and bn.y.dtype == out.dtype:
        lib = _lib.load()
        if bn.slot is not None and few_rows("dgrad_bn", dy.dtype, N, IH, IW, Cin, Cout, KH, stride, pad):
            keep = bn.slot.acquire_bwd()
            part, part_ld = keep
        else:
            rows = stats_rows("dgrad_bn", dy.dtype, N, IH, IW, Cin, Cout, KH, stride, pad)
            keep = part = torch.empty((rows, 2, Cin), dtype=torch.float32, device=dy.device)
            part_ld = 0
        ev = TIMER.span(kernel_name("dgrad_full", dy.dtype, N, IH, IW, Cin, Cout, KH, stride, pad), 2.0 * N * OH * OW * Cout * Cin * KH * KW,
                        nbytes=(dy.numel() + 2 * N * IH * IW * Cin + wT.numel()) * dy.element_size(),
                        shape=("dgrad", N, IH, IW, Cin, Cout, KH, stride)) if TIMER else None
        if ev:
            ev[0].record()
        _lib.check(lib.et_conv2d_dgrad_bn(_lib.ptr(dy), _lib.ptr(wT), _lib.ptr(out), et_dtype(dy), N, IH, IW, Cin, _nhwc(out), Cout,
                                          KH, KW, pad, _nhwc(dy), _lib.ptr(residual), _nhwc(residual) if residual is not None else 0,
                                          _lib.ptr(bn.y), _nhwc(bn.y), _lib.ptr(bn.scale), _lib.ptr(bn.shift), bn.act,
                                          _lib.ptr(part), part_ld, _lib.ptr(zero_page(dy.device)), _lib.stream(dy)), "et_conv2d_dgrad_bn")
        if ev:
            ev[1].record()
        bn.partial, bn.dz_ptr = keep, out.data_ptr()
        return out
    tag = (kernel_name("dgrad_full" if (accumulate or residual is not None) else "dgrad", dy.dtype, N, IH, IW, Cin, Cout, KH, stride, pad) if stride == 1 else
           "conv_gemm (stride-2 dgrad parity classes)") if TIMER else None
    ev = TIMER.span(tag, 2.0 * N * OH * OW * Cout * Cin * KH * KW,
                    stride * stride, nbytes=(dy.numel() + N * IH * IW * Cin + wT.numel()) * dy.element_size(),
                    shape=("dgrad", N, IH, IW, Cin, Cout, KH, stride)) if TIMER else None
    if ev:
        ev[0].record()
    _lib.check(_lib.load().et_conv2d_dgrad(_lib.ptr(dy), _lib.ptr(wT), _lib.ptr(out), et_dtype(dy), N, IH, IW, Cin,
                                           _nhwc(out), Cout, KH, KW, stride, pad, _nhwc(dy), int(accumulate),
                                           _lib.ptr(residual), _nhwc(residual) if residual is not None else 0,
                                           _lib.ptr(zero_page(dy.device)), _lib.stream(dy)), "et_conv2d_dgrad")
    if ev:
        ev[1].record()
    return out


def conv2d_wgrad(x, dy, dw, ksize, stride, pad):
    N, IH, IW, Cin = x.shape
    _, OH, OW, Cout = dy.shape
    assert dw.dtype == torch.float32 and dw.is_contiguous() and dw.shape == (Cout, ksize, ksize, Cin)
    assert x.dtype == dy.dtype
    ev = TIMER.span(kernel_name("wgrad", x.dtype, N, IH, IW, Cin, Cout, ksize, stride, pad), 2.0 * N * OH * OW * Cout * Cin * ksize * ksize) if TIMER else None
    if ev:
        ev[0].record()
    _lib.check(_lib.load().et_conv2d_wgrad(_lib.ptr(x), _lib.ptr(dy), _lib.ptr(dw), et_dtype(x), N, IH, IW, Cin,
                                           _nhwc(x), Cout, ksize, ksize, stride, pad, _nhwc(dy),
                                           _lib.ptr(zero_page(x.device)), _lib.stream(x)), "et_conv2d_wgrad")
    if ev:
        ev[1].record()
    return dw

# ... 587 lines not shown
```

### include/et_hip.h

```cpp
#ifndef ET_HIP_H
#define ET_HIP_H
#include <stddef.h>
#include <stdint.h>

#ifdef __cplusplus
extern "C" {
#endif

typedef void* et_stream_t;

enum { ET_F32 = 0, ET_BF16 = 1, ET_F16 = 2 };

#define ET_ABI_VERSION 7
const char* et_build_arch(void);
int et_abi_version(void);

int et_nms_ssod_workspace_bytes(int B, int A, size_t* bytes );
int et_nms_ssod(const float* pred, int B, int A, int no, float conf_thres, float iou_thres,
                int agnostic, int max_det, float* dets, int* counts, int64_t* keep,
                int* n_candidates, void* workspace, size_t ws_bytes, et_stream_t stream);

int et_nms_workspace_bytes(int B, int A, int no, int multi_label, int max_nms, size_t* bytes );
int et_nms(const float* pred, int B, int A, int no, float conf_thres, float iou_thres, int agnostic,
           int multi_label, uint64_t class_mask_lo, uint64_t class_mask_hi, int max_nms, float max_wh,
           int max_det, float* dets, int* counts, int64_t* keep, int* n_candidates, void* workspace,
           size_t ws_bytes, et_stream_t stream);

int et_val_match(const float* dets, int det_row_stride, const int* counts, int B, int max_det, const float* targets, int NT,
                 const float* shapes, int net_h, int net_w, const float* iouv, int niou, int single_cls, int nc,
                 int64_t row_offset, int64_t arena_rows, int* correct, float* conf, int* cls, int* valid, int* nt,
                 et_stream_t stream);

int et_val_ap_workspace_bytes(int nc, size_t* bytes );
int et_val_ap(const int* cls, const int* correct, const float* conf, int64_t N, const int* nt, int nc, int niou, double* ap,
              double* p, double* r, double* f1, void* workspace, size_t ws_bytes, et_stream_t stream);

int et_detect_decode(const void* raw, int dtype, int B, int na, int ny, int nx, int no,
                     int64_t sb, int64_t sa, int64_t sy, int64_t sx, const float* anchor_px,
                     float stride, float* z, int64_t A_total, int64_t a_offset, et_stream_t stream);

int et_ema_update(float* ema, const float* model, int64_t n, float d, float one_minus_d, et_stream_t stream);
int et_adamw(float* p, const float* grad, float* exp_avg, float* exp_avg_sq, void* lp_shadow, int shadow_dtype, int64_t n, float lr,
             float beta1, float beta2, float eps, float weight_decay, int step, float inv_scale, const float* scaler,
             et_stream_t stream);
int et_adamw_tick(double* tick, float beta1, float beta2, const float* scaler, et_stream_t stream);
int et_adamw_dev(float* p, const float* grad, float* exp_avg, float* exp_avg_sq, void* lp_shadow, int shadow_dtype, int64_t n, float lr,
                 float beta1, float beta2, float eps, float weight_decay, const double* tick, float inv_scale, const float* scaler,
                 et_stream_t stream);
int et_sgd_nesterov(float* p, const float* grad, float* momentum_buf, void* lp_shadow, int shadow_dtype, int64_t n,
                    float lr, float momentum, float weight_decay, int first_step, float inv_scale, const float* scaler,
                    et_stream_t stream);
int et_cast_f32_to_lp(const float* src, void* dst, int dtype, int64_t n, et_stream_t stream);
int et_scaler_check(const float* grads, int64_t n, float* scaler, et_stream_t stream);
int et_scaler_update(float* scaler, float growth_factor, float backoff_factor, int growth_interval, et_stream_t stream);
int et_ema_update_dev(float* ema, const float* model, int64_t n, const float* d_and_one_minus_d, et_stream_t stream);
int et_sgd_nesterov_dev(float* p, const float* grad, float* momentum_buf, void* lp_shadow, int shadow_dtype, int64_t n,
                        const float* hp, int first_step, const float* scaler, et_stream_t stream);

int et_conv2d_stats_rows(int N, int OH, int OW);
int et_conv2d_stats_rows_for(int op, int dtype, int N, int IH, int IW, int Cin, int Cout, int KH, int KW, int stride, int pad,
                             int have_zero_page);
int et_conv2d_stats_adds_for(int op, int dtype, int N, int IH, int IW, int Cin, int Cout, int KH, int KW, int stride, int pad,
                             int have_zero_page);
#define ET_BN_SHARDS 16
int et_conv2d_fwd(const void* x, const void* w, void* y, int dtype, int N, int IH, int IW, int Cin,
                  int ldx, int Cout, int KH, int KW, int stride, int pad, int ldy, const float* scale,
                  const float* bias, int act, const void* residual, int ldr, float* stats_partial, int stats_ld,
                  const void* zero16, et_stream_t stream);
int et_conv2d_dgrad(const void* dy, const void* wT, void* dx, int dtype, int N, int IH, int IW, int Cin,
                    int ldx, int Cout, int KH, int KW, int stride, int pad, int ldy, int accumulate,
                    const void* residual , int ldr,
                    const void* zero16, et_stream_t stream);
int et_conv2d_dgrad_bn(const void* dy, const void* wT, void* dx, int dtype, int N, int IH, int IW, int Cin, int ldx, int Cout,
                       int KH, int KW, int pad, int ldy, const void* residual, int ldr, const void* bn_y, int ld_bn,
                       const float* bn_scale, const float* bn_shift, int bn_act, float* bn_stats_partial,
                       int bn_stats_ld ,
                       const void* zero16, et_stream_t stream);
int et_conv2d_wgrad(const void* x, const void* dy, float* dw, int dtype, int N, int IH, int IW, int Cin,
                    int ldx, int Cout, int KH, int KW, int stride, int pad, int ldy, const void* zero16,
                    et_stream_t stream);
typedef struct et_wgrad_item { const void* x; const void* dy; float* dw; int ldx, ldy; } et_wgrad_item;
int et_conv2d_wgrad_grouped(const et_wgrad_item* items , int n_items, int dtype, int N, int IH, int IW,
                            int Cin, int Cout, int KH, int KW, int stride, int pad, const void* zero16,
                            et_stream_t stream);
int et_weight_transpose(const void* w, void* wT, int dtype, int Cout, int taps, int Cin, et_stream_t stream);
int et_conv2d_kernel_name(int op, int dtype, int N, int IH, int IW, int Cin, int Cout, int KH, int KW, int stride,
                          int pad, int have_zero_page, int parity_class, char* buf , int buflen);
int et_env_knobs(char* buf , int buflen);
int et_weight_transpose_all(const void* w_arena, void* wT_arena, int dtype, const int* table, int n_layers,
                            long long total_elems, et_stream_t stream);
int et_colsum(const void* x, int dtype, int P, int C, int ld, float* out, et_stream_t stream);

int et_bn_reduce_rows(int P, int C, int dtype);
int et_bn_finalize(const float* stats_partial, int rows, int C, double count, const float* gamma,
                   const float* beta, float eps, float momentum, float* running_mean, float* running_var,
                   float* scale, float* shift, float* save_mean, float* save_invstd,
                   double* ws , et_stream_t stream);
int et_bn_eval_affine(int C, const float* gamma, const float* beta, const float* running_mean,
                      const float* running_var, float eps, float* scale, float* shift, et_stream_t stream);
int et_bn_act_fwd(const void* y, int ldy, void* z, int ldz, const void* residual, int ldr, int dtype, int P,
                  int C, const float* scale, const float* shift, int act, et_stream_t stream);
int et_bn_act_bwd(const void* dz, int lddz, const void* y, int ldy, void* dy, int lddy, int dtype, int P, int C,
                  const float* gamma, const float* scale, const float* shift, const float* save_mean,
                  const float* save_invstd, int act, float* dgamma, float* dbeta,
                  double* totals , float* workspace, size_t ws_floats,
                  et_stream_t stream);
int et_bn_act_bwd_from_partials(const void* dz, int lddz, const void* y, int ldy, void* dy, int lddy, int dtype, int P, int C,
                                const float* gamma, const float* scale, const float* shift, const float* save_mean,
                                const float* save_invstd, int act, float* dgamma, float* dbeta, double* totals,
                                const float* partials, int partial_rows, float* workspace, et_stream_t stream);
int et_bn_act_fwd_sharded(const void* y, int ldy, void* z, int ldz, const void* residual, int ldr, int dtype, int P, int C,
                          const float* shards, int shard_ld, double count, const float* gamma, const float* beta, float eps,
                          float momentum, float* running_mean, float* running_var, float* scale, float* shift, float* save_mean,
                          float* save_invstd, int act, et_stream_t stream);
int et_bn_act_bwd_sharded(const void* dz, int lddz, const void* y, int ldy, void* dy, int lddy, int dtype, int P, int C,
                          const float* gamma, const float* scale, const float* shift, const float* save_mean,
                          const float* save_invstd, int act, float* dgamma, float* dbeta, float* shards, int shard_ld, int reduce,
                          et_stream_t stream);
int et_act_bwd(const void* dz, int lddz, const void* y, int ldy, void* dy, int lddy, int dtype, int P, int C,
               int act, et_stream_t stream);

int et_pack_input(const float* x_nchw, void* y_nhwc8, int dtype, int B, int C, int H, int W, et_stream_t stream);
int et_pack_input_u8(const uint8_t* x_nchw, void* y_nhwc8, int dtype, int B, int C, int H, int W, float norm_scale,
                     et_stream_t stream);
int et_maxpool5_fwd(const void* x, int ldx, void* y, int ldy, uint8_t* argmax, int dtype, int B, int H, int W, int C,
                    et_stream_t stream);
int et_maxpool5_bwd(const void* dy, int lddy, const uint8_t* argmax, const void* base, int ldb, void* dx, int lddx,
                    int dtype, int B, int H, int W, int C, et_stream_t stream);
int et_upsample2x_fwd(const void* x, int ldx, void* y, int ldy, int dtype, int B, int H, int W, int C, et_stream_t stream);
int et_upsample2x_bwd(const void* dy, int lddy, void* dx, int lddx, int dtype, int B, int H, int W, int C,
                      int accumulate , et_stream_t stream);

int et_strong_view_u8(const uint8_t* weak, uint8_t* strong, int B, int H, int W, const double* minv, const uint8_t* lut,
                      const int* cutouts, const int* flags, int border_value, et_stream_t stream);
int et_mosaic4_u8(const int64_t* tiles, uint8_t* out, int B, int S, int border_value, et_stream_t stream);

int et_pseudo_label_transform(const float* dets, const int* counts, const double* M_s, int B, int max_det,
                              int width, int height, int clip01 ,
                              double* targets9, uint8_t* valid, et_stream_t stream);
int et_score_log_append(const float* dets, const int* counts, int B, int max_det, float* conf_log, int* cls_log,
                        uint64_t* log_count, int64_t cap, et_stream_t stream);

typedef struct {
    const void* p;
    float* dp;
    void* tobj_ws;
    int64_t sb, sa, sy, sx;
    int ny, nx;
    float anchors[6];
    float balance;
} et_loss_level;
typedef struct {
    int dtype, B, na, nc, NT, nl;
    float anchor_t, gr, cp, cn, cls_pw, obj_pw, box_w, obj_w, cls_w;
    int pass_mask, ignore_obj;
    const float* targets;
    float* acc_ws;
    float* out;
    const int* ota_match;
    int obj_channel;
    float* balance_dev;
    int autobalance_ssi;
    float fl_gamma;
    et_loss_level level[4];
} et_loss_desc;
int et_yolo_loss(const et_loss_desc* desc , et_stream_t stream);
int et_ota_workspace_bytes(int B, int na, int nl, int NT, size_t* bytes);
int et_ota_assign(const et_loss_desc* desc , const float* strides , float img_size, int top_k,
                  void* workspace, int* match, et_stream_t stream);
int et_select_targets(const double* targets9, const uint8_t* valid, int N, const double* thr_low,
                      const double* thr_high, int nc, int with_obj, float* table, et_stream_t stream);
int et_scale_cast(const float* src, void* dst, int dtype, int64_t n, float scale,
                  const float* dev_scale , et_stream_t stream);

int et_domain_focal(const void* feat, int ldf, int dtype, int64_t P, int label, float gscale, void* grad,
                    int ldg, float* loss_sum, et_stream_t stream);
int et_scale_inplace(void* x, int dtype, int64_t n, float alpha, const float* dev_scale ,
                     et_stream_t stream);

int et_v8_decode(const void* reg, int ld_reg, const void* cls, int ld_cls, int dtype, int B, int H, int W, int reg_max, int nc,
                 float stride, float cell_offset, float* out, int64_t A_total, int64_t a_offset, et_stream_t stream);
int et_tal_loss(const float* pred_scores, const float* pred_distri, const float* anchor_points_s, const float* stride_tensor,
                const float* target_bboxes_px, const float* target_scores, const uint8_t* fg_mask, int B, int A, int nc, int reg_max,
                int iou_kind, float w_class, float w_iou, float w_dfl, float* grad_scores, float* grad_distri,
                float* acc_ws , float* out , et_stream_t stream);
int et_tal_assign_workspace_bytes(int B, int A, int G, size_t* bytes );
int et_tal_assign(const float* pd_scores, const float* pd_bboxes, const float* anc_points, const float* gt_labels,
                  const float* gt_bboxes, const float* mask_gt, int B, int A, int G, int nc, int topk, float alpha, float beta,
                  float eps, int64_t* target_labels, float* target_bboxes, float* target_scores, uint8_t* fg_mask,
                  void* workspace, size_t ws_bytes, et_stream_t stream);
int et_tal_targets_pad(const float* targets, int n, int B, int G, float img_w, float img_h, float* out, float* mask, et_stream_t stream);

int et_tal_pseudo_split(const double* targets9, const uint8_t* valid, const double* thr_low, const double* thr_high, int B, int G, int nc,
                        int with_obj, int with_bbox, int with_cls, float img_w, float img_h, float* gt_labels_r, float* gt_bboxes_r,
                        float* gt_labels_u, float* gt_bboxes_u, float* mask_reliable, float* mask_uncertain, float* u_score,
                        uint8_t* u_flags, et_stream_t stream);
int et_tal_assigned_gt(const void* workspace, int B, int A, int G, int32_t* gt_idx, et_stream_t stream);
int et_tal_merge_pseudo(const float* ts_r, const float* tb_r, const uint8_t* fg_r, const float* ts_u, const float* tb_u,
                        const uint8_t* fg_u, const int32_t* gt_idx_u, const float* u_score, const uint8_t* u_flags, int B, int A, int G,
                        int nc, float* target_scores, float* target_bboxes, uint8_t* fg_box, et_stream_t stream);


#ifdef __cplusplus
}
#endif
#endif
```

Before: 1290.

## Fuse uint8 image normalization into stem conv forward and weight-grad kernels

Adds stem conv kernels that read raw uint8 NCHW image segments directly, normalizing through a shared-memory lookup table while staging patches. This removes the separate pack_input pass and its packed bf16 tensor. A dedicated u8 weight-grad kernel also runs on the side stream, so the packed input never has to be materialized or saved for backward. It adds a register-prefetch pipeline and more code paths, and the gain is bounded by how small the stem is within the whole step.

Result: faster. 1309, median of 6 (+1.5%).

```diff
diff --git a/efficientteacher_amd/_lib.py b/efficientteacher_amd/_lib.py
--- a/efficientteacher_amd/_lib.py
+++ b/efficientteacher_amd/_lib.py
@@ -46,6 +46,9 @@
     "et_weight_transpose": (c_int, [P, P, c_int, c_int, c_int, c_int, P]),
     "et_conv2d_kernel_name": (c_int, [c_int] * 13 + [c_char_p, c_int]),
     "et_env_knobs": (c_int, [c_char_p, c_int]),
+    "et_conv2d_stem_u8_fwd": (c_int, [P, P, c_int, c_float, P, P, c_int, c_int, c_int, c_int, c_int, P, P, c_int, P, c_int, P, P]),
+    "et_conv2d_stem_u8_wgrad": (c_int, [P, P, c_int, c_float, P, P, c_int, c_int, c_int, c_int, c_int, P, P]),
+    "et_conv2d_stem_kernel_name": (c_int, [c_int] * 12 + [c_char_p, c_int]),
     "et_colsum": (c_int, [P, c_int, c_int, c_int, c_int, P, P]),
     "et_bn_reduce_rows": (c_int, [c_int, c_int, c_int]),
     "et_bn_finalize": (c_int, [P, c_int, c_int, c_double, P, P, c_float, c_float, P, P, P, P, P, P, P, P]),
@@ -111,7 +114,7 @@
 CALL_TIMER = None
 _NO_LAUNCH = frozenset(n for n in (
     "et_build_arch", "et_abi_version", "et_nms_ssod_workspace_bytes", "et_nms_workspace_bytes", "et_conv2d_stats_rows", "et_conv2d_stats_rows_for",
-    "et_conv2d_kernel_name", "et_env_knobs", "et_bn_reduce_rows", "et_ota_workspace_bytes", "et_tal_assign_workspace_bytes", "et_val_ap_workspace_bytes"))
+    "et_conv2d_kernel_name", "et_conv2d_stem_kernel_name", "et_env_knobs", "et_bn_reduce_rows", "et_ota_workspace_bytes", "et_tal_assign_workspace_bytes", "et_val_ap_workspace_bytes"))
 
 
 class _TimedDll:
diff --git a/efficientteacher_amd/autograd.py b/efficientteacher_amd/autograd.py
--- a/efficientteacher_amd/autograd.py
+++ b/efficientteacher_amd/autograd.py
@@ -144,7 +144,9 @@
 class ConvBnActFn(Function):
 
     @staticmethod
-    def forward(ctx, x, residual, wparam, cs, bs, act, nbt, dst=None, bn_in=None, bn_out=None, acc=None):
+    def forward(ctx, x, residual, wparam, cs, bs, act, nbt, dst=None, bn_in=None, bn_out=None, acc=None, u8=None):
+        ctx.u8 = u8
+        ctx.x_u8 = x if isinstance(x, ops.U8Images) else None
         ctx.w_needs_grad = wparam.requires_grad
         ctx.bn_in = bn_in if (bn_in is not None and cs.stride == 1 and residual is None) else None
         ctx.acc = acc
@@ -159,7 +161,7 @@
         if bn_out is not None and residual is None:
             ctx.bn_mine = _bn_sums(y, scale, shift, act, bs)
             bn_out.append(ctx.bn_mine)
-        ctx.save_for_backward(x, y, scale, shift, mean, invstd)
+        ctx.save_for_backward(None if ctx.x_u8 is not None else x, y, scale, shift, mean, invstd)
         return z
 
     @staticmethod
@@ -168,8 +170,11 @@
         cs, bs = ctx.cs, ctx.bs
         dz = _dense_or_slice(dz)
         dy = _bn_train_bwd(dz, y, bs, scale, shift, mean, invstd, ctx.act, sums=ctx.bn_mine)
-        if ctx.w_needs_grad:
-            _wgrad(x, dy, cs)
+        if ctx.w_needs_grad and ctx.u8 is not None:
+            hook = GRAD_READY_HOOK
+            ops.WGRAD_QUEUE.submit_stem_u8(ctx.u8, dy, cs.gw, on_done=(lambda: hook(cs)) if hook is not None else None)
+        elif ctx.w_needs_grad:
+            _wgrad(x if ctx.x_u8 is None else ctx.x_u8.packed(), dy, cs)
         dx = None
         if ctx.x_needs_grad:
             wT = cs.transposed()
@@ -179,7 +184,7 @@
                 ctx.acc.merged = True
             else:
                 dx = ops.conv2d_dgrad(dy, wT, (x.shape[1], x.shape[2]), cs.stride, cs.pad, bn=_fuse_into(cs, ctx.bn_in, x))
-        return dx, (dz if ctx.has_res else None), None, None, None, None, None, None, None, None, None
+        return dx, (dz if ctx.has_res else None), None, None, None, None, None, None, None, None, None, None
 
 
 class BottleneckFn(Function):
diff --git a/efficientteacher_amd/csrc/conv.hip b/efficientteacher_amd/csrc/conv.hip
--- a/efficientteacher_amd/csrc/conv.hip
+++ b/efficientteacher_amd/csrc/conv.hip
@@ -1537,6 +1537,7 @@
 #define STEM_PSLOTS (7 * 256)
 #define STEM_WPITCH 37
 #define STEM_WSLOTS (10 * 256)
+#define STEM_MAX_SEGS 4
 
 struct StemArgs {
     const uint16_t* x; const uint16_t* w; uint16_t* y; const uint16_t* zero;
@@ -1545,15 +1546,32 @@
     const float* scale; const float* bias; int act;
     float* stats; int stat_rows;
     int stats_ld;
+    const uint8_t* seg[STEM_MAX_SEGS]; int seg_b[STEM_MAX_SEGS]; float norm;
 };
 
-template <typename T, int ACT>
-__global__ __launch_bounds__(256, 2) void conv_stem_kernel(StemArgs a) {
+template <typename A> __device__ __forceinline__ const uint8_t* stem_u8_image(const A& a, int n) {
+    const uint8_t* p = a.seg[0];
+    int b = 0;
+#pragma unroll
+    for (int s = 1; s < STEM_MAX_SEGS; ++s)
+        if (n >= a.seg_b[s]) { p = a.seg[s]; b = a.seg_b[s]; }
+    return p + (size_t)(n - b) * 3 * a.IH * a.IW;
+}
+template <typename T> __device__ __forceinline__ void stem_u8_fill_lut(uint16_t* lut, int tid, float norm) {
+    lut[tid] = (uint16_t)(et_lp<T>::pack((float)((unsigned)tid & 0xffu) / norm, 0.f) & 0xffffu);
+}
+
+#define STEM_QPR 34
+#define STEM_NQ (STEM_PH * STEM_QPR)
+template <typename T, int ACT, bool U8>
+__device__ __forceinline__ void conv_stem_body(const StemArgs& a) {
     __shared__ __attribute__((aligned(16))) u32x4 wl[STEM_WSLOTS];
     __shared__ __attribute__((aligned(16))) u32x4 pl[STEM_PSLOTS];
+    __shared__ uint16_t lut[U8 ? 256 : 2];
     const int tid = threadIdx.x, lane = tid & 63;
     const int wave = __builtin_amdgcn_readfirstlane(tid >> 6);
     const int l31 = lane & 31, hi = lane >> 5;
+    if constexpr (U8) stem_u8_fill_lut<T>(lut, tid, a.norm);
 
 #pragma unroll
     for (int i = 0; i < STEM_WSLOTS / 256; ++i) {
@@ -1602,13 +1620,61 @@
             et_glds16(src, pl + i * 256 + wave * 64);
         }
     };
-    if ((int)blockIdx.x < a.ntiles) stage_patch(blockIdx.x);
+    int q_row[2], q_col[2];
+    unsigned q_px[2][3];
+    bool q_in[2];
+#pragma unroll
+    for (int i = 0; i < 2; ++i) {
+        const int q = i * 256 + tid;
+        q_row[i] = q < STEM_NQ ? q / STEM_QPR : -100000;
+        q_col[i] = q % STEM_QPR;
+        q_in[i] = false;
+#pragma unroll
+        for (int c = 0; c < 3; ++c) q_px[i][c] = 0u;
+    }
+    auto load_u8 = [&](int tile) {
+        const int tc = tile % a.tcn, t2 = tile / a.tcn;
+        const int tr = t2 % a.trn, n = t2 / a.trn;
+        const int iy0 = 2 * tr * STEM_TR - 2, ix0 = 2 * tc * STEM_TC - 4;
+        const uint8_t* const img = stem_u8_image(a, n);
+#pragma unroll
+        for (int i = 0; i < 2; ++i) {
+            const int iy = iy0 + q_row[i], ix = ix0 + 4 * q_col[i];
+            q_in[i] = (unsigned)iy < (unsigned)a.IH && (unsigned)ix < (unsigned)a.IW;
+#pragma unroll
+            for (int c = 0; c < 3; ++c)
+                q_px[i][c] = q_in[i] ? *(const unsigned*)(img + ((size_t)c * a.IH + iy) * a.IW + ix) : 0u;
+        }
+    };
+    auto write_patch_u8 = [&]() {
+#pragma unroll
+        for (int i = 0; i < 2; ++i)
+#pragma unroll
+            for (int j = 0; j < 4; ++j) {
+                const int pc = 4 * q_col[i] - 2 + j;
+                if (q_row[i] >= 0 && (unsigned)pc < (unsigned)STEM_PITCH) {
+                    const unsigned r = lut[(q_px[i][0] >> (8 * j)) & 0xffu], g = lut[(q_px[i][1] >> (8 * j)) & 0xffu];
+                    const unsigned b = lut[(q_px[i][2] >> (8 * j)) & 0xffu];
+                    pl[q_row[i] * STEM_PITCH + pc] = q_in[i] ? mk4(r | (g << 16), b, 0u, 0u) : mk4(0u, 0u, 0u, 0u);
+                }
+            }
+    };
+    if constexpr (U8) {
+        __syncthreads();
+        if ((int)blockIdx.x < a.ntiles) load_u8(blockIdx.x);
+    } else {
+        if ((int)blockIdx.x < a.ntiles) stage_patch(blockIdx.x);
+    }
     for (int tile = blockIdx.x; tile < a.ntiles; tile += gridDim.x) {
         const int tc = tile % a.tcn, t2 = tile / a.tcn;
         const int tr = t2 % a.trn, n = t2 / a.trn;
         const int oy0 = tr * STEM_TR, ox0 = tc * STEM_TC;
+        if constexpr (U8) write_patch_u8();
         et_wait_vmem();
         __syncthreads();
+        if constexpr (U8) {
+            if (tile + (int)gridDim.x < a.ntiles) load_u8(tile + gridDim.x);
+        }
         f32x16 acc[2][2];
 #pragma unroll
         for (int cb = 0; cb < 2; ++cb)
@@ -1630,7 +1696,9 @@
                     acc[cb][pb] = et_mfma32<T>(wf[cb], pf[pb], acc[cb][pb]);
         }
         __syncthreads();
-        if (tile + (int)gridDim.x < a.ntiles) stage_patch(tile + gridDim.x);
+        if constexpr (!U8) {
+            if (tile + (int)gridDim.x < a.ntiles) stage_patch(tile + gridDim.x);
+        }
         const int oy = oy0 + wave;
 #pragma unroll
         for (int pb = 0; pb < 2; ++pb) {
@@ -1700,6 +1768,10 @@
         }
     }
 }
+template <typename T, int ACT>
+__global__ __launch_bounds__(256, 2) void conv_stem_kernel(StemArgs a) { conv_stem_body<T, ACT, false>(a); }
+template <typename T, int ACT>
+__global__ __launch_bounds__(256, 2) void conv_stem_u8_kernel(StemArgs a) { conv_stem_body<T, ACT, true>(a); }
 
 static int env_int(const char* name, int dflt) { const char* e = getenv(name); return e ? atoi(e) : dflt; }
 static int device_cus() {
@@ -2130,6 +2202,175 @@
                 }
             }
     }
+}
+
+#define SWG_PITCH 136
+#define SWG_DYV (256 * 8)
+struct StemWgradArgs {
+    const uint8_t* seg[STEM_MAX_SEGS]; int seg_b[STEM_MAX_SEGS]; float norm;
+    const uint16_t* dy; const uint16_t* zero; float* dw;
+    int N, IH, IW, OH, OW, ldy, Cout;
+    int trn, tcn, ntiles;
+};
+
+template <typename T>
+__global__ __launch_bounds__(256, 2) void conv_stem_u8_wgrad_kernel(StemWgradArgs a) {
+    __shared__ __attribute__((aligned(16))) u32x4 dyl[2 * SWG_DYV];
+    __shared__ __attribute__((aligned(16))) u32x4 xl[STEM_PH * SWG_PITCH / 2];
+    __shared__ uint16_t lut[256];
+    const int tid = threadIdx.x, lane = tid & 63;
+    const int wave = __builtin_amdgcn_readfirstlane(tid >> 6);
+    const int l31 = lane & 31, hi = lane >> 5;
+    stem_u8_fill_lut<T>(lut, tid, a.norm);
+
+    int q_row[2], q_col[2];
+    unsigned q_px[2][3];
+    bool q_in[2];
+#pragma unroll
+    for (int i = 0; i < 2; ++i) {
+        const int q = i * 256 + tid;
+        q_row[i] = q < STEM_NQ ? q / STEM_QPR : -100000;
+        q_col[i] = q % STEM_QPR;
+        q_in[i] = false;
+#pragma unroll
+        for (int c = 0; c < 3; ++c) q_px[i][c] = 0u;
+    }
+    auto load_u8 = [&](int tile) {
+        const int tc = tile % a.tcn, t2 = tile / a.tcn;
+        const int tr = t2 % a.trn, n = t2 / a.trn;
+        const int iy0 = 2 * tr * STEM_TR - 2, ix0 = 2 * tc * STEM_TC - 4;
+        const uint8_t* const img = stem_u8_image(a, n);
+#pragma unroll
+        for (int i = 0; i < 2; ++i) {
+            const int iy = iy0 + q_row[i], ix = ix0 + 4 * q_col[i];
+            q_in[i] = (unsigned)iy < (unsigned)a.IH && (unsigned)ix < (unsigned)a.IW;
+#pragma unroll
+            for (int c = 0; c < 3; ++c)
+                q_px[i][c] = q_in[i] ? *(const unsigned*)(img + ((size_t)c * a.IH + iy) * a.IW + ix) : 0u;
+        }
+    };
+    auto write_patch = [&]() {
+#pragma unroll
+        for (int i = 0; i < 2; ++i) {
+            if (q_row[i] < 0) continue;
+            unsigned w[8];
+#pragma unroll
+            for (int j = 0; j < 4; ++j) {
+                const unsigned r = lut[(q_px[i][0] >> (8 * j)) & 0xffu], g = lut[(q_px[i][1] >> (8 * j)) & 0xffu];
+                const unsigned b = lut[(q_px[i][2] >> (8 * j)) & 0xffu];
+                w[2 * j] = q_in[i] ? (r | (g << 16)) : 0u;
+                w[2 * j + 1] = q_in[i] ? b : 0u;
+            }
+            u32x4* const d = xl + (q_row[i] * SWG_PITCH + 4 * q_col[i]) / 2;
+            d[0] = mk4(w[0], w[1], w[2], w[3]);
+            d[1] = mk4(w[4], w[5], w[6], w[7]);
+        }
+    };
+    auto stage_dy = [&](int tile, int buf) {
+        const int tc = tile % a.tcn, t2 = tile / a.tcn;
+        const int tr = t2 % a.trn, n = t2 / a.trn;
+        const int oy0 = tr * STEM_TR, ox0 = tc * STEM_TC;
+#pragma unroll
+        for (int i = 0; i < 8; ++i) {
+            const int slot = i * 256 + tid, p = slot >> 3;
+            const int co = ((slot & 7) ^ tr_swz<8>(p)) * 8;
+            const int oy = oy0 + (p >> 6), ox = ox0 + (p & 63);
+            const bool ok = oy < a.OH && ox < a.OW && co < a.Cout;
+            const uint16_t* src = ok ? a.dy + ((((size_t)n * a.OH + oy) * a.OW + ox) * a.ldy + co) : a.zero;
+            et_glds16(src, dyl + buf * SWG_DYV + i * 256 + wave * 64);
+        }
+    };
+
+    const int fp = 8 * hi + ((lane & 15) >> 2);
+    const int fc = 16 * ((lane >> 4) & 1) + 4 * (lane & 3);
+    int boff[5];
+#pragma unroll
+    for (int nb = 0; nb < 5; ++nb) {
+        const int tap = min(8 * nb + 4 * ((lane >> 4) & 1) + (lane & 3), 35);
+        const int ky = tap / 6, kx = tap - 6 * ky;
+        boff[nb] = (((2 * wave + ky) * SWG_PITCH) + kx + 2 + 2 * fp) * 8;
+    }
+    f32x16 acc[2][5];
+#pragma unroll
+    for (int mb = 0; mb < 2; ++mb)
+#pragma unroll
+        for (int nb = 0; nb < 5; ++nb)
+#pragma unroll
+            for (int r = 0; r < 16; ++r) acc[mb][nb][r] = 0.f;
+
+    __syncthreads();
+    if ((int)blockIdx.x < a.ntiles) { load_u8(blockIdx.x); stage_dy(blockIdx.x, 0); }
+    int it = 0;
+    for (int tile = blockIdx.x; tile < a.ntiles; tile += gridDim.x, ++it) {
+        write_patch();
+        et_wait_vmem();
+        __syncthreads();
+        if (tile + (int)gridDim.x < a.ntiles) { load_u8(tile + gridDim.x); stage_dy(tile + gridDim.x, (it + 1) & 1); }
+        const char* const ta = (const char*)(dyl + (it & 1) * SWG_DYV);
+        const char* const tb = (const char*)xl;
+#pragma unroll
+        for (int ks = 0; ks < 4; ++ks) {
+            s16x8 af[2], bf[5];
+#pragma unroll
+            for (int r = 0; r < 2; ++r) {
+                const int p = wave * 64 + 16 * ks + 4 * r + fp;
+#pragma unroll
+                for (int mb = 0; mb < 2; ++mb) {
+                    const int ch = mb * 32 + fc;
+                    const int off = (p * 8 + ((ch >> 3) ^ tr_swz<8>(p))) * 16 + (ch & 4) * 2;
+                    const s16x4 v = __builtin_amdgcn_ds_read_tr16_b64_v4i16((__attribute__((address_space(3))) s16x4*)(ta + off));
+                    af[mb][4 * r + 0] = v[0]; af[mb][4 * r + 1] = v[1]; af[mb][4 * r + 2] = v[2]; af[mb][4 * r + 3] = v[3];
+                }
+#pragma unroll
+                for (int nb = 0; nb < 5; ++nb) {
+                    const int off = boff[nb] + 2 * (16 * ks + 4 * r) * 8;
+                    const s16x4 v = __builtin_amdgcn_ds_read_tr16_b64_v4i16((__attribute__((address_space(3))) s16x4*)(tb + off));
+                    bf[nb][4 * r + 0] = v[0]; bf[nb][4 * r + 1] = v[1]; bf[nb][4 * r + 2] = v[2]; bf[nb][4 * r + 3] = v[3];
+                }
+            }
+#pragma unroll
+            for (int mb = 0; mb < 2; ++mb)
+#pragma unroll
+                for (int nb = 0; nb < 5; ++nb)
+                    acc[mb][nb] = et_mfma32<T>(af[mb], bf[nb], acc[mb][nb]);
+        }
+        __syncthreads();
+    }
+    et_wait_vmem();
+    float* const red = (float*)dyl;
+#pragma unroll 1
+    for (int w = 1; w < 4; ++w) {
+        __syncthreads();
+        if (wave == w) {
+#pragma unroll
+            for (int mb = 0; mb < 2; ++mb)
+#pragma unroll
+                for (int nb = 0; nb < 5; ++nb)
+#pragma unroll
+                    for (int r = 0; r < 16; ++r) red[((mb * 5 + nb) * 16 + r) * 64 + lane] = acc[mb][nb][r];
+        }
+        __syncthreads();
+        if (wave == 0) {
+#pragma unroll
+            for (int mb = 0; mb < 2; ++mb)
+#pragma unroll
+                for (int nb = 0; nb < 5; ++nb)
+#pragma unroll
+                    for (int r = 0; r < 16; ++r) acc[mb][nb][r] += red[((mb * 5 + nb) * 16 + r) * 64 + lane];
+        }
+    }
+    if (wave != 0 || (l31 & 3) == 3) return;
+#pragma unroll
+    for (int mb = 0; mb < 2; ++mb)
+#pragma unroll
+        for (int r = 0; r < 16; ++r) {
+            const int co = mb * 32 + 8 * (r >> 2) + 4 * hi + (r & 3);
+#pragma unroll
+            for (int nb = 0; nb < 5; ++nb) {
+                const int tap = 8 * nb + (l31 >> 2);
+                if (co < a.Cout && tap < 36) atomicAdd(a.dw + ((size_t)co * 36 + tap) * 8 + (l31 & 3), acc[mb][nb][r]);
+            }
+        }
 }
 
 template <typename T, int BM, int BNC, int WM, int WN, int STRIDE = 1>
@@ -3054,6 +3295,85 @@
     return 0;
 }
 
+static int stem_u8_mode(int dtype, int in_is_u8, int C, int IW, int Cout, int KH, int KW, int stride, int pad) {
+    if (!in_is_u8 || C != 3 || (dtype != ET_BF16 && dtype != ET_F16) || KH != 6 || KW != 6 || stride != 2 || pad != 2 || IW % 4 ||
+        Cout > 64 || Cout % 8 || Cout < 8)
+        return 0;
+    return env_int("ET_STEM_U8", 3) & 3;
+}
+template <typename A>
+static int stem_u8_segments(A& a, const void* const* seg_ptrs, const int* seg_counts, int n_segs, int IH, int IW) {
+    if (!seg_ptrs || !seg_counts || n_segs < 1 || n_segs > STEM_MAX_SEGS || IH < 1 || IW < 4 || IW % 4) return -2;
+    int n = 0;
+    for (int s = 0; s < STEM_MAX_SEGS; ++s) {
+        a.seg[s] = s < n_segs ? (const uint8_t*)seg_ptrs[s] : (const uint8_t*)seg_ptrs[0];
+        a.seg_b[s] = s < n_segs ? n : 0x7fffffff;
+        if (s < n_segs) {
+            if (seg_counts[s] < 1 || !seg_ptrs[s] || ((uintptr_t)seg_ptrs[s] & 3)) return -2;
+            n += seg_counts[s];
+        }
+    }
+    if ((long long)n * 3 * IH * IW >= (1ll << 40)) return -2;
+    return n;
+}
+
+extern "C" int et_conv2d_stem_u8_fwd(const void* const* seg_ptrs, const int* seg_counts, int n_segs, float norm_scale, const void* w,
+                                     void* y, int dtype, int IH, int IW, int Cout, int ldy, const float* scale, const float* bias,
+                                     int act, float* stats, int stats_ld, const void* zero16, et_stream_t stream) {
+    if (!w || !y || !zero16 || !(stem_u8_mode(dtype, 1, 3, IW, Cout, 6, 6, 2, 2) & 1) || ldy < Cout || ldy % 8 || act < 0 || act > 2) return -2;
+    StemArgs a;
+    const int N = stem_u8_segments(a, seg_ptrs, seg_counts, n_segs, IH, IW);
+    if (N < 0) return N;
+    a.norm = norm_scale;
+    a.x = nullptr; a.zero = (const uint16_t*)zero16;
+    a.w = (const uint16_t*)w; a.y = (uint16_t*)y;
+    a.N = N; a.IH = IH; a.IW = IW; a.ldx = 8; a.Cout = Cout; a.ldy = ldy;
+    a.OH = (IH + 4 - 6) / 2 + 1; a.OW = (IW + 4 - 6) / 2 + 1;
+    if (a.OH < 1 || a.OW < 1) return -2;
+    a.trn = (a.OH + STEM_TR - 1) / STEM_TR; a.tcn = (a.OW + STEM_TC - 1) / STEM_TC;
+    a.ntiles = N * a.trn * a.tcn;
+    a.scale = scale; a.bias = bias; a.act = act; a.stats = stats; a.stats_ld = stats ? stats_ld : 0;
+    a.stat_rows = (N * a.OH * a.OW + 63) / 64;
+    int grid = env_int("ET_CONV_STEM_WGS", 2 * device_cus());
+    if (grid < 1) grid = 1;
+    if (grid > a.ntiles) grid = a.ntiles;
+    if (stats && !stats_ld && grid > a.stat_rows) grid = a.stat_rows;
+    hipStream_t s = (hipStream_t)stream;
+#define ET_STEM(T_) \
+    do { \
+        if (act == ACT_SILU) hipLaunchKernelGGL((conv_stem_u8_kernel<T_, ACT_SILU>), dim3(grid), dim3(256), 0, s, a); \
+        else if (act == ACT_RELU) hipLaunchKernelGGL((conv_stem_u8_kernel<T_, ACT_RELU>), dim3(grid), dim3(256), 0, s, a); \
+        else hipLaunchKernelGGL((conv_stem_u8_kernel<T_, ACT_NONE>), dim3(grid), dim3(256), 0, s, a); \
+    } while (0)
+    if (dtype == ET_F16) ET_STEM(et_f16); else ET_STEM(uint16_t);
+#undef ET_STEM
+    ET_CHECK_LAUNCH();
+    return 0;
+}
+
+extern "C" int et_conv2d_stem_u8_wgrad(const void* const* seg_ptrs, const int* seg_counts, int n_segs, float norm_scale, const void* dy,
+                                       float* dw, int dtype, int IH, int IW, int Cout, int ldy, const void* zero16, et_stream_t stream) {
+    if (!dy || !dw || !zero16 || !(stem_u8_mode(dtype, 1, 3, IW, Cout, 6, 6, 2, 2) & 2) || ldy < Cout || ldy % 8 || ((uintptr_t)dy & 15)) return -2;
+    StemWgradArgs a;
+    const int N = stem_u8_segments(a, seg_ptrs, seg_counts, n_segs, IH, IW);
+    if (N < 0) return N;
+    a.norm = norm_scale;
+    a.dy = (const uint16_t*)dy; a.zero = (const uint16_t*)zero16; a.dw = dw;
+    a.N = N; a.IH = IH; a.IW = IW; a.ldy = ldy; a.Cout = Cout;
+    a.OH = (IH + 4 - 6) / 2 + 1; a.OW = (IW + 4 - 6) / 2 + 1;
+    if (a.OH < 1 || a.OW < 1) return -2;
+    a.trn = (a.OH + STEM_TR - 1) / STEM_TR; a.tcn = (a.OW + STEM_TC - 1) / STEM_TC;
+    a.ntiles = N * a.trn * a.tcn;
+    int grid = env_int("ET_CONV_STEM_WGS", 2 * device_cus());
+    if (grid < 1) grid = 1;
+    if (grid > a.ntiles) grid = a.ntiles;
+    hipStream_t s = (hipStream_t)stream;
+    if (dtype == ET_F16) hipLaunchKernelGGL((conv_stem_u8_wgrad_kernel<et_f16>), dim3(grid), dim3(256), 0, s, a);
+    else hipLaunchKernelGGL((conv_stem_u8_wgrad_kernel<uint16_t>), dim3(grid), dim3(256), 0, s, a);
+    ET_CHECK_LAUNCH();
+    return 0;
+}
+
 extern "C" int et_conv2d_kernel_name(int op, int dtype, int N, int IH, int IW, int Cin, int Cout, int KH, int KW, int stride,
                                      int pad, int have_zero_page, int parity_class, char* buf, int buflen) {
     if (!buf || buflen < 8) return -1;
@@ -3086,8 +3406,17 @@
     return 0;
 }
 
+extern "C" int et_conv2d_stem_kernel_name(int op, int dtype, int in_is_u8, int C, int N, int IH, int IW, int Cout, int KH, int KW, int stride,
+                                          int pad, char* buf, int buflen) {
+    if (!buf || buflen < 32 || (op != 0 && op != 2)) return -1;
+    const int mode = stem_u8_mode(dtype, in_is_u8, C, IW, Cout, KH, KW, stride, pad);
+    if (op == 0 && (mode & 1)) { snprintf(buf, buflen, "conv_stem_u8_kernel"); return 0; }
+    if (op == 2 && (mode & 2)) { snprintf(buf, buflen, "conv_stem_u8_wgrad_kernel<%s>", dtype == ET_F16 ? "et_f16" : "unsigned short"); return 0; }
+    return et_conv2d_kernel_name(op, dtype, N, IH, IW, 8, Cout, KH, KW, stride, pad, 1, 0, buf, buflen);
+}
+
 extern "C" int et_env_knobs(char* buf, int buflen) {
-    static const char* names[] = {"ET_CONV_S1_WGS", "ET_CONV_STEM_WGS", "ET_CONV_BUF_DMA", "ET_BN_FIN_SMALL", "ET_STEP_GRAPH", "ET_WGRAD_STREAM",
+    static const char* names[] = {"ET_CONV_S1_WGS", "ET_CONV_STEM_WGS", "ET_CONV_BUF_DMA", "ET_BN_FIN_SMALL", "ET_STEP_GRAPH", "ET_WGRAD_STREAM", "ET_STEM_U8",
                                   "ET_ALLREDUCE_CHUNK_MB", "ET_ALLREDUCE_DTYPE", "ET_RCCL_CHANNELS", "ET_DP_SINGLE_RANK", "ET_HIP_LIB"};
     if (!buf || buflen < 1) return -1;
     int off = 0;
diff --git a/efficientteacher_amd/models/backbone/common.py b/efficientteacher_amd/models/backbone/common.py
--- a/efficientteacher_amd/models/backbone/common.py
+++ b/efficientteacher_amd/models/backbone/common.py
@@ -50,9 +50,15 @@
                                "(model.to('cuda')) before calling it -- there is no CPU path")
         bs = self.bn._et_slot
         act = _act_code(self.act)
+        u8 = None
+        if isinstance(x, ops.U8Images):
+            mode = ops.stem_u8_mode(x, cs.w_lp, cs.stride, cs.pad)
+            u8 = x if mode & 2 else None
+            if not mode & 1:
+                x = x.packed()
         if self.bn.training:
             nbt = None if self._et_flat().bulk_nbt else self.bn.num_batches_tracked
-            return ConvBnActFn.apply(x, residual, self.conv.weight, cs, bs, act, nbt, dst, bn_in, bn_out, acc)
+            return ConvBnActFn.apply(x, residual, self.conv.weight, cs, bs, act, nbt, dst, bn_in, bn_out, acc, u8)
         flat = self._et_flat()
         o = bs.aff_off
         out = None if dst is None else dst[0][..., dst[1]:dst[1] + cs.coutp]
diff --git a/efficientteacher_amd/models/backbone/yolov5_backbone.py b/efficientteacher_amd/models/backbone/yolov5_backbone.py
--- a/efficientteacher_amd/models/backbone/yolov5_backbone.py
+++ b/efficientteacher_amd/models/backbone/yolov5_backbone.py
@@ -18,6 +18,7 @@
 
 
 class YoloV5BackBone(nn.Module):
+    reads_u8_images = True
     supports_concat_dst = True
 
     def __init__(self, cfg):
diff --git a/efficientteacher_amd/models/detector/yolo.py b/efficientteacher_amd/models/detector/yolo.py
--- a/efficientteacher_amd/models/detector/yolo.py
+++ b/efficientteacher_amd/models/detector/yolo.py
@@ -157,7 +157,11 @@
         flat.prepare_forward(self.training)
         if not all(t.dim() == 4 and t.shape[1] <= 8 for t in (x if isinstance(x, (list, tuple)) else (x,))):
             raise ValueError("expected an NCHW image batch (B, 3, H, W), or a list of such batches of one shape")
-        x8 = ops.pack_input(x, self._compute_dtype, norm_scale=getattr(self, "input_norm_scale", 255.0))
+        norm = getattr(self, "input_norm_scale", 255.0)
+        if getattr(self.backbone, "reads_u8_images", False):
+            x8 = ops.stem_input(x, self._compute_dtype, norm_scale=norm)
+        else:
+            x8 = ops.pack_input(x, self._compute_dtype, norm_scale=norm)
         slots = None
         if (hasattr(self.neck, "concat_slots") and getattr(self.backbone, "supports_concat_dst", False)
                 and x8.shape[1] % 32 == 0 and x8.shape[2] % 32 == 0):
diff --git a/efficientteacher_amd/ops.py b/efficientteacher_amd/ops.py
--- a/efficientteacher_amd/ops.py
+++ b/efficientteacher_amd/ops.py
@@ -35,7 +35,7 @@
 
     FAMILY = {
         "et_conv2d_fwd": "gather_gemm", "et_conv2d_dgrad": "gather_gemm", "et_conv2d_dgrad_bn": "gather_gemm",
-        "et_conv2d_wgrad": "wgrad", "et_conv2d_wgrad_grouped": "wgrad",
+        "et_conv2d_wgrad": "wgrad", "et_conv2d_wgrad_grouped": "wgrad", "et_conv2d_stem_u8_fwd": "gather_gemm", "et_conv2d_stem_u8_wgrad": "wgrad",
         "et_bn_finalize": "bn", "et_bn_act_fwd": "bn", "et_bn_act_fwd_sharded": "bn", "et_bn_act_bwd_sharded": "bn", "et_bn_act_bwd": "bn", "et_bn_act_bwd_from_partials": "bn", "et_act_bwd": "bn",
         "et_nms": "nms_loss_pl", "et_nms_ssod": "nms_loss_pl", "et_detect_decode": "nms_loss_pl", "et_pseudo_label_transform": "nms_loss_pl",
         "et_select_targets": "nms_loss_pl", "et_yolo_loss": "nms_loss_pl", "et_ota_assign": "nms_loss_pl", "et_score_log_append": "nms_loss_pl",
@@ -165,7 +165,116 @@
     return (ih + 2 * p - k) // s + 1, (iw + 2 * p - k) // s + 1
 
 
+class U8Images:
+    requires_grad = False
+    is_cuda = True
+
+    def __init__(self, parts, dtype, norm_scale):
+        self.parts = [p.contiguous() for p in parts]
+        _, C, H, W = self.parts[0].shape
+        assert all(p.dtype == torch.uint8 and p.shape[1:] == (C, H, W) and p.device == self.parts[0].device for p in self.parts)
+        self.C = C
+        self.shape = torch.Size((sum(p.shape[0] for p in self.parts), H, W, 8))
+        self.dtype, self.device, self.norm_scale = dtype, self.parts[0].device, float(norm_scale)
+        self._packed = None
+
+    def dim(self):
+        return 4
+
+    def packed(self):
+        if self._packed is None:
+            self._packed = pack_input(self.parts, self.dtype, self.norm_scale)
+        return self._packed
+
+    def c_segments(self):
+        n = len(self.parts)
+        import ctypes
+        ptrs = (ctypes.c_void_p * n)(*[_lib.ptr(p) for p in self.parts])
+        counts = (ctypes.c_int * n)(*[p.shape[0] for p in self.parts])
+        return ptrs, counts, n
+
+
+STEM_MAX_SEGS = 4
+
+
+def stem_kernel_name(op, dtype, in_is_u8, C, N, IH, IW, Cout, k, stride, pad):
+    import ctypes
+    buf = ctypes.create_string_buffer(256)
+    _lib.check(_lib.load().et_conv2d_stem_kernel_name({"fwd": 0, "wgrad": 2}[op], _ET_OF[dtype], int(bool(in_is_u8)), C, N, IH, IW, Cout,
+                                                      k, k, stride, pad, buf, 256), "et_conv2d_stem_kernel_name")
+    return buf.value.decode()
+
+
+def stem_input(x, dtype, norm_scale=255.0):
+    parts = list(x) if isinstance(x, (list, tuple)) else [x]
+    if (dtype in LP_DTYPES and len(parts) <= STEM_MAX_SEGS
+            and all(p.dtype == torch.uint8 and p.dim() == 4 and p.shape[1] == 3 and p.shape[3] % 4 == 0 and (p.is_cuda or _lib.is_emulated())
+                    and p.shape[0] > 0 and p.shape[1:] == parts[0].shape[1:] for p in parts)):
+        u8 = U8Images(parts, dtype, norm_scale)
+        if all(p.data_ptr() % 4 == 0 for p in u8.parts):
+            return u8
+    return pack_input(x, dtype, norm_scale=norm_scale)
+
+
+def stem_u8_mode(u8, w, stride, pad):
+    N, IH, IW, _ = u8.shape
+    Cout, KH, KW, Cin = w.shape
+    if KH != KW or Cin != 8:
+        return 0
+    a = (u8.dtype, True, u8.C, N, IH, IW, Cout, KH, stride, pad)
+    return (1 if stem_kernel_name("fwd", *a) == "conv_stem_u8_kernel" else 0) | \
+           (2 if stem_kernel_name("wgrad", *a).startswith("conv_stem_u8_wgrad_kernel") else 0)
+
+
+def _stem_u8_fwd(u8, w, stride, pad, scale, bias, act, out, want_stats, shards):
+    N, IH, IW, _ = u8.shape
+    Cout = w.shape[0]
+    assert w.is_contiguous() and w.dtype == u8.dtype and tuple(w.shape[1:]) == (6, 6, 8) and stride == 2 and pad == 2
+    OH, OW = conv_out_hw(IH, IW, 6, 2, 2)
+    if out is None:
+        out = torch.empty((N, OH, OW, Cout), dtype=u8.dtype, device=u8.device)
+    assert out.shape == (N, OH, OW, Cout)
+    stats, stats_ld = None, 0
+    if shards is not None:
+        assert not want_stats
+        stats, stats_ld = shards
+    if want_stats:
+        stats = torch.empty((stats_rows("fwd", u8.dtype, N, IH, IW, 8, Cout, 6, 2, 2), 2, Cout), dtype=torch.float32, device=u8.device)
+    ev = TIMER.span("conv_stem_u8_kernel", 2.0 * N * OH * OW * Cout * 3 * 36,
+                    nbytes=N * 3 * IH * IW + (N * OH * OW * Cout + w.numel()) * w.element_size(),
+                    shape=("fwd", N, IH, IW, 3, Cout, 6, 2)) if TIMER else None
+    if ev:
+        ev[0].record()
+    ptrs, counts, n = u8.c_segments()
+    _lib.check(_lib.load().et_conv2d_stem_u8_fwd(ptrs, counts, n, u8.norm_scale, _lib.ptr(w), _lib.ptr(out), et_dtype(w), IH, IW, Cout,
+                                                 _nhwc(out), _lib.ptr(scale), _lib.ptr(bias), act, _lib.ptr(stats), stats_ld,
+                                                 _lib.ptr(zero_page(u8.device)), _lib.stream(out)), "et_conv2d_stem_u8_fwd")
+    if ev:
+        ev[1].record()
+    return (out, stats) if want_stats else out
+
+
+def stem_u8_wgrad(u8, dy, dw):
+    N, IH, IW, _ = u8.shape
+    _, OH, OW, Cout = dy.shape
+    assert dy.dtype == u8.dtype and dy.shape[:3] == (N,) + conv_out_hw(IH, IW, 6, 2, 2)
+    assert dw.dtype == torch.float32 and dw.is_contiguous() and dw.shape == (Cout, 6, 6, 8)
+    ev = TIMER.span(stem_kernel_name("wgrad", u8.dtype, True, 3, N, IH, IW, Cout, 6, 2, 2), 2.0 * N * OH * OW * Cout * 3 * 36, 1,
+                    nbytes=N * 3 * IH * IW + N * OH * OW * Cout * dy.element_size() + 8 * Cout * 108,
+                    shape=("wgrad", N, IH, IW, 3, Cout, 6, 2)) if TIMER else None
+    if ev:
+        ev[0].record()
+    ptrs, counts, n = u8.c_segments()
+    _lib.check(_lib.load().et_conv2d_stem_u8_wgrad(ptrs, counts, n, u8.norm_scale, _lib.ptr(dy), _lib.ptr(dw), et_dtype(dy), IH, IW, Cout,
+                                                   _nhwc(dy), _lib.ptr(zero_page(dy.device)), _lib.stream(dy)), "et_conv2d_stem_u8_wgrad")
+    if ev:
+        ev[1].record()
+
+
 def conv2d_fwd(x, w, stride, pad, *, scale=None, bias=None, act=ACT_NONE, residual=None, out=None, want_stats=False, shards=None):
+    if isinstance(x, U8Images):
+        assert residual is None
+        return _stem_u8_fwd(x, w, stride, pad, scale, bias, act, out, want_stats, shards)
     N, IH, IW, Cin = x.shape
     Cout, KH, KW, Cin2 = w.shape
     assert Cin == Cin2 and w.is_contiguous() and w.dtype == x.dtype
@@ -246,6 +355,31 @@
         self.last[key] = self.tick
         if len(lst) >= self.group:
             self._flush_key(key)
+
+    def submit_stem_u8(self, u8, dy, dw, on_done=None):
+        dev = dy.device
+        side_ok = dev.type == "cuda" and self.use_side in (1, 3)
+        if side_ok and not self._cb_armed:
+            try:
+                torch.autograd.Variable._execution_engine.queue_callback(self.flush)
+                self._cb_armed = True
+            except RuntimeError:
+                side_ok = False
+        if side_ok:
+            main, side = torch.cuda.current_stream(dev), self.side_stream(dev)
+            side.wait_stream(main)
+            with torch.cuda.stream(side):
+                stem_u8_wgrad(u8, dy, dw)
+                dy.record_stream(side)
+                for p in u8.parts:
+                    p.record_stream(side)
+                if on_done is not None:
+                    on_done()
+            self._dirty.add(dev)
+            return
+        stem_u8_wgrad(u8, dy, dw)
+        if on_done is not None:
+            on_done()
 
     def _flush_key(self, key):
         lst = self.pending.pop(key, None)
diff --git a/include/et_hip.h b/include/et_hip.h
--- a/include/et_hip.h
+++ b/include/et_hip.h
@@ -11,7 +11,7 @@
 
 enum { ET_F32 = 0, ET_BF16 = 1, ET_F16 = 2 };
 
-#define ET_ABI_VERSION 7
+#define ET_ABI_VERSION 8
 const char* et_build_arch(void);
 int et_abi_version(void);
 
@@ -87,6 +87,13 @@
 int et_conv2d_kernel_name(int op, int dtype, int N, int IH, int IW, int Cin, int Cout, int KH, int KW, int stride,
                           int pad, int have_zero_page, int parity_class, char* buf , int buflen);
 int et_env_knobs(char* buf , int buflen);
+int et_conv2d_stem_u8_fwd(const void* const* seg_ptrs, const int* seg_counts, int n_segs, float norm_scale, const void* w, void* y,
+                          int dtype, int IH, int IW, int Cout, int ldy, const float* scale, const float* bias, int act,
+                          float* stats_partial, int stats_ld, const void* zero16, et_stream_t stream);
+int et_conv2d_stem_u8_wgrad(const void* const* seg_ptrs, const int* seg_counts, int n_segs, float norm_scale, const void* dy, float* dw,
+                            int dtype, int IH, int IW, int Cout, int ldy, const void* zero16, et_stream_t stream);
+int et_conv2d_stem_kernel_name(int op, int dtype, int in_is_u8, int C, int N, int IH, int IW, int Cout, int KH, int KW, int stride,
+                               int pad, char* buf , int buflen);
 int et_weight_transpose_all(const void* w_arena, void* wT_arena, int dtype, const int* table, int n_layers,
                             long long total_elems, et_stream_t stream);
 int et_colsum(const void* x, int dtype, int P, int C, int ld, float* out, et_stream_t stream);
```
